# Runki2018/litehandnet

Hardware: AMD Instinct MI355X
Metric: images/sec fwd+bwd @256x256 bs64 litehandnet (higher is better)
Workload: dtype f32; 1 GPU; litehandnet variant B (MSRB hourglass litehourglass.py) C=128, 256x256x3 -> 21x64x64, per-GPU batch 64, train-mode BN, fwd + TopdownHeatmapLoss + bwd + fused Adam; global_batch=64, parallelism=dp1

## Files before the change

### include/lhn.h

```cpp
#ifndef LHN_H
#define LHN_H
#include <stdint.h>
#ifdef __cplusplus
extern "C" {
#endif

#define LHN_VERSION 3
#define LHN_STAT_REPLICAS 32

typedef struct lhn_view {
  float*       data;
  const float* table;
  const float* gate;
  int32_t N, H, W;
  int32_t cstride;
  int32_t coff;
  int32_t C;
  const void* pend;
} lhn_view;

typedef struct lhn_gradview {
  const float* dz;
  const float* dpool;
  const float* coef;
// ... 170 lines not shown
int lhn_shuffle2_fwd(const lhn_view* a, const lhn_view* b, const lhn_view* dst, void* stream);
int lhn_shuffle2_bwd(const lhn_view* a, const lhn_view* b, const lhn_view* dst, const float* ddst, float* da, int acc_a,
                     float* db, int acc_b, void* stream);
int lhn_maxpool2_fwd(const lhn_view* x, const lhn_view* y, void* stream);
int lhn_avgpool_fwd(const lhn_view* x, float* out , int OH, int OW, void* stream);
int lhn_avgpool_fwd2(const lhn_view* x, float* out, int OH, int OW, int out_cstride, int out_coff, void* stream);
int lhn_avgpool_bwd2(const lhn_view* x, const float* dout, int OH, int OW, int out_cstride, int out_coff, float* dx,
                     int dx_accumulate, void* stream);
int lhn_ca_mlp_fwd(const float* pooled , const float* w3 , const float* gamma,
                   const float* beta, float* rmean, float* rvar, int64_t* nbt, const float* w1 ,
                   const float* b1, const float* w2 , const float* b2, const float* dropmask,
                   float* gate, int gate_stride, int gate_coff, float* save , int N, int C,
                   float eps, float momentum, int training, int stage, double* gsum, double count_scale,
                   void* stream);

int lhn_att_mlp_fwd(const float* pooled, const float* gamma, const float* beta, float* rmean, float* rvar,
                    int64_t* nbt, const float* w3 , const float* b3, const float* wl ,
                    const float* bl, const float* dropmask , float* gate, int gate_stride,
                    int gate_coff, float* save, int N, int C, float eps, float momentum, int training, int stage,
                    double* gsum, double count_scale, void* stream);
int lhn_att_mlp_bwd(const float* pooled, const float* gamma, const float* beta, const float* w3, const float* wl,
                    const float* dropmask, float* save, const float* dgate , float* dpool, int cstride,
                    int coff, int H, int W, float* dgamma, float* dbeta, float* dw3, float* db3, float* dwl,
                    float* dbl, int N, int C, int stage, double* gsum, double count_scale, float pgrad_scale,
                    void* stream);

int lhn_se_mlp_fwd(const float* pooled, const float* w1 , const float* b1, const float* w2 ,
                   const float* b2, float* gate, int gate_stride, int gate_coff, float* save, int N, int C, int J,
                   void* stream);
int lhn_se_mlp_fwd2(const float* pooled, const float* w1, const float* b1, const float* w2, const float* b2, float* gate,
                    int gate_stride, int gate_coff, float* save, int N, int C, int J, int mode, void* stream);
int lhn_se_mlp_bwd2(const float* pooled, const float* w1, const float* w2, const float* save, const float* dgate,
                    float* dpool, int cstride, int coff, int H, int W, float* dw1, float* db1, float* dw2, float* db2, int N,
                    int C, int J, int mode, void* stream);
int lhn_se_mlp_bwd(const float* pooled, const float* w1, const float* w2, const float* save, const float* dgate ,
                   float* dpool , int cstride, int coff, int H, int W, float* dw1, float* db1, float* dw2,
                   float* db2, int N, int C, int J, void* stream);

int lhn_bn_bwd_reduce(const lhn_view* y, const lhn_gradview* g, const float* save_mean_invstd,
                      double* sums , const lhn_bnbwdfin* fin , void* stream);
int lhn_bn_bwd_finalize(const double* sums, const float* gamma, const float* save_mean_invstd,
                        float* coef, int cstride, int coff, int C, double count, float* dgamma, float* dbeta,
                        float pgrad_scale , void* stream);
int lhn_bn_bwd_finalize2(const double* sums, const float* gamma, const float* save_mean_invstd, float* coef, int cstride,
                         int coff, int C, int stat_channels, double count, float* dgamma, float* dbeta, float pgrad_scale,
                         void* stream);
int lhn_conv_pw_bwd(const lhn_view* x, const float* w, const lhn_view* y, const lhn_gradview* gy,
                    float* dx , int dx_accumulate, float* dw,
                    float* dbias, int stride, const float* dy_nchw, int nrep, int64_t rep_stride, void* stream);
int lhn_conv_pw_bwd2(const lhn_view* x, const float* w, const lhn_view* y, const lhn_gradview* gy, float* dx,
                     int dx_accumulate, float* dw, float* dbias, int stride, const float* dy_nchw, int nrep, int64_t rep_stride,
                     const lhn_pw_opts* opts, void* stream);
int lhn_conv_dw_bwd(const lhn_view* x, const float* w, const lhn_view* y, const lhn_gradview* gy, float* dx,
                    int dx_accumulate, float* dw, int k, int stride, int pad, int dil, int nrep, int64_t rep_stride,
                    void* stream);
int lhn_conv_dw_bwd2(const lhn_view* x, const float* w, const lhn_view* y, const lhn_gradview* gy, float* dx, int dx_accumulate,
                     float* dw, int k, int stride, int pad, int dil, int nrep, int64_t rep_stride, double* bn_sums,
                     const float* bn_save, int bn_C, int bn_coff, void* stream);
int lhn_conv_dw_bwd3(const lhn_view* x, const float* w, const lhn_view* y, const lhn_gradview* gy, float* dx, int dx_accumulate,
                     float* dw, int k, int stride, int pad, int dil, int nrep, int64_t rep_stride, const float* dx_add0,
                     const float* dx_add1, void* stream);
int lhn_conv_stem_bwd(const float* img, const lhn_view* y, const lhn_gradview* gy, float* dw, int Hi, int Wi,
                      int k, int stride, int pad, int nrep, int64_t rep_stride, void* stream);
int lhn_conv_kxk_bwd(const lhn_view* x, const float* w, const lhn_view* y, const lhn_gradview* gy, float* dx,
                     int dx_accumulate, float* dw, int stride, int nrep, int64_t rep_stride,
                     float* wt_scratch , void* stream);
int lhn_plan_run_range(void* plan, int phase, int64_t step_begin, int64_t step_end, void* workspace,
                       void* const* params, void* const* grads, void* const* io, int training, int grad_replicas,
                       int64_t grad_rep_stride, double count_scale, float pgrad_scale, void* stream);
int lhn_fold_stat_replicas(double* stats, int64_t n, int nrep, void* stream);
int lhn_reduce_replicas(float* out, const float* part, int64_t n, int nrep, int64_t rep_stride, void* stream);
int lhn_ew_bwd(const lhn_view* srcs, int nsrc, const lhn_view* dst, const float* ddst, float out_slope,
               float* const* dsrcs, const int* accumulate, void* stream);
int lhn_ew_bwd2(const lhn_view* src, const lhn_view* dst, const float* ddst, const float* dst_dpool, float out_slope,
                float* dsrc, int accumulate, void* stream);
int lhn_maxpool2_bwd(const lhn_view* x, const lhn_view* y, const float* dy, float* dx, int dx_accumulate,
                     void* stream);
int lhn_maxpool2_bwd2(const lhn_view* x, const lhn_view* y, const float* dy, float* dx, int dx_accumulate, const lhn_bnsum* bns,
                      void* stream);
int lhn_maxpool2_bwd3(const lhn_view* x, const lhn_view* y, const float* dy, float* dx, int dx_accumulate, const lhn_bnsum* bns,
                      const lhn_grad_adds* adds , void* stream);
int lhn_ew_bwd3(const lhn_view* src, const lhn_view* dst, const float* ddst, const float* dst_dpool, float out_slope, float* dsrc,
                int accumulate, const lhn_bnsum* bns, void* stream);
int lhn_ew_bwd_multi(const lhn_view* srcs, int nsrc, const lhn_view* dst, const float* ddst, const float* dst_dpool, float out_slope,
                     float* const* dsrcs, const int* accumulate, const lhn_bnsum* const* bns, void* stream);
int lhn_avgpool_bwd3(const lhn_view* x, const float* dout, int OH, int OW, int out_cstride, int out_coff, float* dx,
                     int dx_accumulate, const lhn_bnsum* bns, void* stream);
int lhn_conv_pw_bwd3(const lhn_view* x, const float* w, const lhn_view* y, const lhn_gradview* gy, float* dx, int dx_accumulate,
                     float* dw, float* dbias, int stride, const float* dy_nchw, int nrep, int64_t rep_stride,
                     const lhn_pw_opts* opts, const lhn_bnsum* bns , void* stream);
int lhn_conv_dw_bwd4(const lhn_view* x, const float* w, const lhn_view* y, const lhn_gradview* gy, float* dx, int dx_accumulate,
                     float* dw, int k, int stride, int pad, int dil, int nrep, int64_t rep_stride, const lhn_bnsum* bns,
                     const float* dx_add0, const float* dx_add1, const lhn_bnbwdsrc* fin, void* stream);
int lhn_conv_pw_bwd4(const lhn_view* x, const float* w, const lhn_view* y, const lhn_gradview* gy, float* dx, int dx_accumulate,
                     float* dw, float* dbias, int stride, const float* dy_nchw, int nrep, int64_t rep_stride,
                     const lhn_pw_opts* opts, const lhn_bnsum* bns, const lhn_bnbwdsrc* fin, void* stream);
int lhn_avgpool_bwd(const lhn_view* x, const float* dout , int OH, int OW, float* dx,
                    int dx_accumulate, void* stream);
int lhn_gate_bwd_reduce(const lhn_view* y, const float* dz, float* dgate , void* stream);
typedef struct lhn_bn_slices {
  const float* save[2];
  double*      sums[2];
  int32_t      lo[2], C[2];
  int32_t      n;
} lhn_bn_slices;
int lhn_gate_bwd_reduce2(const lhn_view* y, const float* dz, float* dgate , float* tsum,
                         const lhn_bn_slices* slices, void* stream);
int lhn_gate_bwd_reduce3(const lhn_view* y, const float* dz, float* dgate, float* tsum, const lhn_bn_slices* slices, int prezeroed,
                         void* stream);
typedef struct lhn_gatesum {
  float*               dgate;
  const lhn_bn_slices* slices;
} lhn_gatesum;
int lhn_conv_pw_bwd5(const lhn_view* x, const float* w, const lhn_view* y, const lhn_gradview* gy, float* dx, int dx_accumulate,
                     float* dw, float* dbias, int stride, const float* dy_nchw, int nrep, int64_t rep_stride,
                     const lhn_pw_opts* opts, const lhn_bnsum* bns, const lhn_bnbwdsrc* fin, const lhn_gatesum* gs, void* stream);
int lhn_avgpool_fwd3(const lhn_view* x, float* out , int OH, int OW, float* pstat ,
                     const lhn_bn_slices* slices, void* stream);
int lhn_ca_mlp_bwd2(const float* pooled, const float* w3, const float* gamma, const float* w1, const float* w2,
                    const float* dropmask, const float* save, const float* dgate, float* dpool, int cstride, int coff, int H,
                    int W, float* dw3, float* dgamma, float* dbeta, float* dw1, float* db1, float* dw2, float* db2, int N, int C,
                    int stage, double* gsum, double count_scale, float pgrad_scale, const float* tsum, const float* pstat,
                    const lhn_bn_slices* slices, void* stream);
int lhn_avgpool_fwd4(const lhn_view* x, float* out, int OH, int OW, float* pstat, const lhn_bn_slices* slices,
                     const lhn_view* copy_src, void* stream);
int lhn_ca_mlp_bwd(const float* pooled, const float* w3, const float* gamma, const float* w1, const float* w2,
                   const float* dropmask, const float* save, const float* dgate, float* dpool ,
                   int cstride, int coff, int H, int W, float* dw3, float* dgamma, float* dbeta, float* dw1,
                   float* db1, float* dw2, float* db2, int N, int C, int stage, double* gsum, double count_scale,
                   float pgrad_scale, void* stream);

int lhn_cbam_layout(int N, int H, int W, int C, int64_t* save_off , int64_t* scratch_off );
int lhn_cbam_fwd(const lhn_view* p, const lhn_view* r, const float* w1, const float* w2, const float* w7, const lhn_view* out,
                 float* save, void* stream);
int lhn_cbam_bwd(const lhn_view* p, const lhn_view* r, const float* w1, const float* w2, const float* w7, const lhn_view* out,
                 const float* dout, float* dp, float* dr, float* dw1, float* dw2, float* dw7, const float* save, float* scratch,
                 void* stream);

int lhn_adam_step(float* param, const float* grad, float* exp_avg, float* exp_avg_sq, int64_t n, double lr, double beta1,
                  double beta2, double eps, double weight_decay, int64_t step, void* stream);

typedef struct lhn_op {
  int32_t kind;
  int32_t in_buf[3], in_coff[3], in_C[3];
  int32_t reserved[6];
  int32_t out_buf, out_coff, out_C;
  int32_t p[12];
  int64_t ws[12];
  int32_t i[8];
  float   f[8];
} lhn_op;

typedef struct lhn_buf {
  int64_t data_off, table_off, gate_off, grad_off, dpool_off, coef_off;
  int32_t N, H, W, C;
} lhn_buf;

void* lhn_plan_create(const lhn_buf* bufs, int nbufs, const lhn_op* fwd, int nfwd, const lhn_op* bwd, int nbwd);
void  lhn_plan_destroy(void* plan);
int   lhn_plan_head_gate_fold(void* plan);
#define LHN_RUN_TABLES_CURRENT 2
#define LHN_RUN_GRAPH 4
int   lhn_plan_run(void* plan, int phase, void* workspace, void* const* params, void* const* grads,
                   void* const* io, int training, int grad_replicas, int64_t grad_rep_stride, void* stream);

#ifdef __cplusplus
}
#endif
#endif
```

### litehandnet_amd/_lib.py

```python
import ctypes as C
import os

import torch

_HERE = os.path.dirname(os.path.abspath(__file__))
LIB_PATH = os.path.join(_HERE, "liblhn.so")
_lib = None


class LhnError(RuntimeError):
    pass


class View(C.Structure):
    _fields_ = [("data", C.c_void_p), ("table", C.c_void_p), ("gate", C.c_void_p),
                ("N", C.c_int32), ("H", C.c_int32), ("W", C.c_int32),
                ("cstride", C.c_int32), ("coff", C.c_int32), ("C", C.c_int32), ("pend", C.c_void_p)]


class GradView(C.Structure):
    _fields_ = [("dz", C.c_void_p), ("dpool", C.c_void_p), ("coef", C.c_void_p)]


class Op(C.Structure):
    _fields_ = [("kind", C.c_int32),
                ("in_buf", C.c_int32 * 3), ("in_coff", C.c_int32 * 3), ("in_C", C.c_int32 * 3), ("reserved", C.c_int32 * 6),
                ("out_buf", C.c_int32), ("out_coff", C.c_int32), ("out_C", C.c_int32),
                ("p", C.c_int32 * 12), ("ws", C.c_int64 * 12), ("i", C.c_int32 * 8), ("f", C.c_float * 8)]


class Buf(C.Structure):
    _fields_ = [("data_off", C.c_int64), ("table_off", C.c_int64), ("gate_off", C.c_int64),
                ("grad_off", C.c_int64), ("dpool_off", C.c_int64), ("coef_off", C.c_int64),
                ("N", C.c_int32), ("H", C.c_int32), ("W", C.c_int32), ("C", C.c_int32)]


SYMBOLS = [
    "lhn_version", "lhn_deterministic", "lhn_last_error", "lhn_device_ok",
    "lhn_heatmap_encode", "lhn_heatmap_argmax", "lhn_heatmap_refine", "lhn_transform_preds",
    "lhn_heatmap_decode", "lhn_heatmap_decode_dark", "lhn_heatmap_decode_dark_udp", "lhn_heatmap_nms", "lhn_heatmap_topk", "lhn_pck_accuracy",
    "lhn_eval_state_bytes", "lhn_eval_accumulate", "lhn_eval_finalize",
    "lhn_loss_balanced_mse_fwd", "lhn_loss_balanced_mse_bwd", "lhn_affine_warp_normalize", "lhn_affine_warp_normalize2", "lhn_random_flip", "lhn_hsv_jitter", "lhn_simdr_encode", "lhn_simdr_loss_fwd", "lhn_simdr_loss_bwd",
    "lhn_conv_pw_fwd", "lhn_conv_pw_fwd2", "lhn_conv_pw_bwd2", "lhn_conv_dw_fwd", "lhn_conv_dw_fwd2", "lhn_conv_dw_fwd3", "lhn_conv_pw_dw3_fwd", "lhn_conv_dw3_pw_fwd", "lhn_msrb_round_scratch_bytes", "lhn_msrb_round_fwd", "lhn_bottleneck_fwd", "lhn_conv_stem_fwd", "lhn_conv_kxk_fwd",
    "lhn_bn_finalize", "lhn_table_fill", "lhn_table_bias", "lhn_fold_bn", "lhn_ew_fwd", "lhn_ew_fwd2", "lhn_ew_fwd3", "lhn_ew_mul_bwd", "lhn_bilinear_bwd", "lhn_shuffle2_fwd", "lhn_shuffle2_bwd", "lhn_bn_finalize2", "lhn_bn_bwd_finalize2", "lhn_maxpool2_fwd", "lhn_avgpool_fwd", "lhn_avgpool_fwd2", "lhn_avgpool_bwd2", "lhn_se_mlp_fwd2", "lhn_se_mlp_bwd2", "lhn_ca_mlp_fwd", "lhn_att_mlp_fwd", "lhn_att_mlp_bwd", "lhn_se_mlp_fwd", "lhn_se_mlp_bwd",
    "lhn_bn_bwd_reduce", "lhn_bn_bwd_finalize", "lhn_conv_pw_bwd", "lhn_conv_dw_bwd", "lhn_conv_dw_bwd2", "lhn_conv_dw_bwd3", "lhn_conv_dw_bwd4", "lhn_conv_pw_bwd4", "lhn_conv_pw_bwd5", "lhn_plan_head_gate_fold", "lhn_conv_stem_bwd",
    "lhn_conv_kxk_bwd", "lhn_ew_bwd", "lhn_ew_bwd2", "lhn_maxpool2_bwd", "lhn_maxpool2_bwd2", "lhn_maxpool2_bwd3", "lhn_ew_bwd3", "lhn_ew_bwd_multi", "lhn_avgpool_bwd3", "lhn_conv_pw_bwd3", "lhn_avgpool_bwd", "lhn_gate_bwd_reduce", "lhn_gate_bwd_reduce2", "lhn_gate_bwd_reduce3", "lhn_adam_step", "lhn_avgpool_fwd3", "lhn_avgpool_fwd4", "lhn_ca_mlp_bwd2",
    "lhn_ca_mlp_bwd", "lhn_reduce_replicas", "lhn_fold_stat_replicas", "lhn_plan_create", "lhn_plan_destroy", "lhn_plan_run", "lhn_plan_run_range",
    "lhn_cbam_layout", "lhn_cbam_fwd", "lhn_cbam_bwd",
]


def lib():
    global _lib
    if _lib is None:
        if not os.path.exists(LIB_PATH):
            raise LhnError(f"{LIB_PATH} is missing: run `python -m litehandnet_amd.build` "
                           "(hipcc --offload-arch=gfx950); there is no CPU fallback")
        _lib = C.CDLL(LIB_PATH)
        _lib.lhn_last_error.restype = C.c_char_p
        _lib.lhn_plan_create.restype = C.c_void_p
        _lib.lhn_plan_destroy.restype = None
        _lib.lhn_eval_state_bytes.restype = C.c_int64
        _lib.lhn_conv_dw3_pw_fwd.argtypes = [C.c_void_p, C.c_void_p, C.c_int, C.c_void_p, C.c_void_p, C.c_void_p, C.c_void_p, C.c_void_p]
        _lib.lhn_conv_dw3_pw_fwd.restype = C.c_int
        _lib.lhn_msrb_round_scratch_bytes.argtypes = [C.c_int, C.c_int, C.c_int, C.c_int]
        _lib.lhn_msrb_round_scratch_bytes.restype = C.c_int64
        _lib.lhn_msrb_round_fwd.argtypes = [C.c_void_p, C.c_void_p, C.c_void_p, C.c_void_p, C.c_void_p, C.c_void_p, C.c_void_p, C.c_int, C.c_int,
                                            C.c_void_p, C.c_void_p]
        _lib.lhn_msrb_round_fwd.restype = C.c_int
        _lib.lhn_bottleneck_fwd.argtypes = [C.c_void_p, C.c_int] + [C.c_void_p] * 8 + [C.c_float, C.c_void_p, C.c_void_p, C.c_void_p]
        _lib.lhn_bottleneck_fwd.restype = C.c_int
        _lib.lhn_cbam_layout.argtypes = [C.c_int, C.c_int, C.c_int, C.c_int, C.c_void_p, C.c_void_p]
        _lib.lhn_cbam_layout.restype = C.c_int
        _lib.lhn_cbam_fwd.argtypes = [C.c_void_p] * 8
        _lib.lhn_cbam_fwd.restype = C.c_int
        _lib.lhn_cbam_bwd.argtypes = [C.c_void_p] * 15
        _lib.lhn_cbam_bwd.restype = C.c_int
    return _lib


def cbam_layout(N, H, W, Cc):
    sv, sc = (C.c_int64 * 10)(), (C.c_int64 * 8)()
    check(lib().lhn_cbam_layout(N, H, W, Cc, sv, sc), "lhn_cbam_layout")
    return list(sv), list(sc)


def check(status, what=""):
    if status != 0:
        raise LhnError(f"{what}: status {status}: {lib().lhn_last_error().decode()}")


def require_device(t=None):
    if not torch.cuda.is_available():
        raise LhnError("no GPU visible: litehandnet_amd has no CPU fallback")
    if t is not None and not t.is_cuda:
        raise LhnError("tensor must live on the GPU (litehandnet_amd has no CPU fallback)")


def ptr(t):
    return C.c_void_p(0) if t is None else C.c_void_p(t.data_ptr())


def stream():
    return C.c_void_p(torch.cuda.current_stream().cuda_stream)


def f32c(t, name="tensor"):
    require_device(t)
    if t.dtype != torch.float32:
        t = t.float()
    return t.contiguous()
```

### litehandnet_amd/csrc/k_conv_head.hip

```cpp
#include <stdlib.h>
#include "lhn_common.h"

bool lhn_head_stream_on() {
  static int v = -1;
  if (v < 0) {
    const char* e = getenv("LHN_HEAD_STREAM");
    v = (e && e[0] == '0') ? 0 : 1;
  }
  return v == 1;
}

constexpr int HCIN = 128, HLDX = HCIN + 4;
constexpr int HLDR = HCIN + 8;

__global__ void __launch_bounds__(256, 2) k_head_fwd(lhn_view x, const float* __restrict__ w, const float* __restrict__ bias,
                                                     float* __restrict__ y_nchw, int cout, int M, int HoWo, int ntiles, int64_t bstride) {
  constexpr int BM = 128, C4 = HCIN / 4, RP = 256 / C4, PF = BM / RP;
  extern __shared__ __attribute__((aligned(16))) float smem[];
  const int tid = threadIdx.x, lane = tid & 63, wave = __builtin_amdgcn_readfirstlane(tid >> 6), l31 = lane & 31, lh = lane >> 5;
  const int co = l31;
  float wreg[HCIN / 2];
#pragma unroll
  for (int kc = 0; kc < HCIN / 8; ++kc) {
    f4 v = (f4){0.f, 0.f, 0.f, 0.f};
    if (co < cout) v = *reinterpret_cast<const f4*>(w + (int64_t)co * HCIN + kc * 8 + 4 * lh);
    wreg[kc * 4 + 0] = v.x; wreg[kc * 4 + 1] = v.y; wreg[kc * 4 + 2] = v.z; wreg[kc * 4 + 3] = v.w;
  }
  const float bv = (bias && co < cout) ? bias[co] : 0.f;
  const int c4 = tid % C4, row0 = tid / C4, cabs = x.coff + 4 * c4;
  const bool uni = HoWo % BM == 0;
  const f4 one4 = (f4){1.f, 1.f, 1.f, 1.f};
  f4 pre[PF], gpre = one4;
  auto issue = [&](int tile) __attribute__((always_inline)) {
#pragma unroll
    for (int p = 0; p < PF; ++p) {
      const int m = min(tile * BM + row0 + p * RP, M - 1);
      pre[p] = *reinterpret_cast<const f4*>(x.data + (int64_t)m * x.cstride + cabs);
    }
    if (uni) gpre = x.gate ? *reinterpret_cast<const f4*>(x.gate + (int64_t)(min(tile * BM, M - 1) / HoWo) * x.cstride + cabs) : one4;
  };
  int tile = blockIdx.x;
  if (tile < ntiles) issue(tile);
  const Xf4 xf = lhn_load_xf(x, cabs);
  for (; tile < ntiles; tile += gridDim.x) {
#pragma unroll
    for (int p = 0; p < PF; ++p) {
      const int row = row0 + p * RP, m = tile * BM + row;
      f4 g = gpre;
      if (!uni) g = x.gate ? *reinterpret_cast<const f4*>(x.gate + (int64_t)(min(m, M - 1) / HoWo) * x.cstride + cabs) : one4;
      const f4 v = lhn_apply_xf(pre[p], xf) * g;
      *reinterpret_cast<f4*>(smem + row * HLDX + 4 * c4) = m < M ? v : (f4){0.f, 0.f, 0.f, 0.f};
    }
    __syncthreads();
    if (tile + (int)gridDim.x < ntiles) issue(tile + gridDim.x);
    f16v acc;
#pragma unroll
    for (int r = 0; r < 16; ++r) acc[r] = 0.f;
    const float* arow = smem + (wave * 32 + l31) * HLDX + 4 * lh;
#pragma unroll
    for (int kc = 0; kc < HCIN / 8; ++kc) {
      const f4 a = *reinterpret_cast<const f4*>(arow + kc * 8);
      acc = __builtin_amdgcn_mfma_f32_32x32x2f32(a.x, wreg[kc * 4 + 0], acc, 0, 0, 0);
      acc = __builtin_amdgcn_mfma_f32_32x32x2f32(a.y, wreg[kc * 4 + 1], acc, 0, 0, 0);
      acc = __builtin_amdgcn_mfma_f32_32x32x2f32(a.z, wreg[kc * 4 + 2], acc, 0, 0, 0);
      acc = __builtin_amdgcn_mfma_f32_32x32x2f32(a.w, wreg[kc * 4 + 3], acc, 0, 0, 0);
    }
    __syncthreads();
    if (co < cout) {
      const int mbase = tile * BM + wave * 32 + 4 * lh;
#pragma unroll
      for (int g = 0; g < 4; ++g) {
        const int m0 = mbase + 8 * g;
        if (m0 < M) {
          const int n = m0 / HoWo, p = m0 - n * HoWo;
          *reinterpret_cast<f4*>(y_nchw + (int64_t)n * bstride + (int64_t)co * HoWo + p) =
              (f4){acc[4 * g] + bv, acc[4 * g + 1] + bv, acc[4 * g + 2] + bv, acc[4 * g + 3] + bv};
        }
      }
    }
  }
}

int lhn_head_fwd(const lhn_view* x, const float* w, const float* bias, float* y_nchw, int cout, int HoWo, int64_t bstride, hipStream_t s) {
  const int M = x->N * HoWo, ntiles = (M + 127) / 128;
  const size_t lds = (size_t)128 * HLDX * sizeof(float);
  static LhnKernelCfg cfg;
  int per_cu = 1;
  if (!lhn_kernel_cfg(cfg, &k_head_fwd, lds, 2, &per_cu)) {
    lhn_set_error("lhn_conv_pw_fwd: cannot reserve %zu B of LDS", lds);
    return 2;
  }
  int grid = lhn_num_cus() * per_cu;
  if (grid > ntiles) grid = ntiles;
  hipLaunchKernelGGL(k_head_fwd, dim3(grid), dim3(256), lds, s, *x, w, bias, y_nchw, cout, M, HoWo, ntiles, bstride);
  return 0;
}

struct HeadGate {
  float* dgate;
  float* tsum;
  const float* save[2];
  int lo[2], C[2], n;
};

template <bool GS>
__global__ void __launch_bounds__(256, 2) k_head_bwd(lhn_view x, const float* __restrict__ w, const float* __restrict__ dy,
                                                     float* __restrict__ dx, int dx_acc, float* __restrict__ dw, float* __restrict__ dbias,
                                                     int cout, int M, int HoWo, int ntiles, int chunk, int64_t bstride, int nrep,
                                                     int64_t rep_stride, HeadGate hg) {
  constexpr int PX = 64, LDY = 36, XC4 = HCIN / 4, XRP = 256 / XC4, XPF = PX / XRP;
  extern __shared__ __attribute__((aligned(16))) float smem[];
  float* dYs = smem;
  float* Xs = dYs + PX * LDY;
  float* Xr = Xs + PX * HLDX;
  const int tid = threadIdx.x, lane = tid & 63, wave = __builtin_amdgcn_readfirstlane(tid >> 6), l31 = lane & 31, lh = lane >> 5;
  const int xc4 = tid % XC4, xr0 = tid / XC4, xabs = x.coff + 4 * xc4;
  const int yr4 = tid & 15, yco = tid >> 4;
  const bool uni = HoWo % PX == 0;
  const f4 one4 = (f4){1.f, 1.f, 1.f, 1.f}, zero4 = (f4){0.f, 0.f, 0.f, 0.f};
  f4 xraw[XPF], yraw[2], gpre = one4;
  auto issue = [&](int tile) __attribute__((always_inline)) {
#pragma unroll
    for (int p = 0; p < XPF; ++p) {
      const int m = min(tile * PX + xr0 + p * XRP, M - 1);
      xraw[p] = *reinterpret_cast<const f4*>(x.data + (int64_t)m * x.cstride + xabs);
    }
    const int m4 = min(tile * PX + 4 * yr4, M - 4);
    const int n = m4 / HoWo, p = m4 - n * HoWo;
#pragma unroll
    for (int k = 0; k < 2; ++k)
      yraw[k] = yco + 16 * k < cout ? *reinterpret_cast<const f4*>(dy + (int64_t)n * bstride + (int64_t)(yco + 16 * k) * HoWo + p) : zero4;
    if (uni) gpre = x.gate ? *reinterpret_cast<const f4*>(x.gate + (int64_t)(min(tile * PX, M - 1) / HoWo) * x.cstride + xabs) : one4;
  };
  const int t0 = blockIdx.x * chunk, t1 = min(ntiles, t0 + chunk);
  if (t0 < t1) issue(t0);
  const Xf4 xf = lhn_load_xf(x, xabs);
  float wreg[16];
#pragma unroll
  for (int k = 0; k < 16; ++k) {
    const int co = (k >> 2) * 8 + 4 * lh + (k & 3);
    wreg[k] = (dx && co < cout) ? w[(int64_t)co * HCIN + 32 * wave + l31] : 0.f;
  }
  f16v accw;
#pragma unroll
  for (int r = 0; r < 16; ++r) accw[r] = 0.f;
  double bsum[2] = {0.0, 0.0};
  const int cg = x.coff + 32 * wave + l31;
  float g_sc = 1.f, g_sh = 0.f, g_sl = 1.f, g_mean = 0.f, g_inv = 1.f, g_d = 0.f, g_0 = 0.f, g_1 = 0.f;
  int n_cur = -1;
  if (GS) {
    if (x.table) {
      g_sc = x.table[cg];
      g_sh = x.table[x.cstride + cg];
      g_sl = x.table[2 * x.cstride + cg];
    }
#pragma unroll
    for (int k = 0; k < 2; ++k)
      if (k < hg.n && cg >= hg.lo[k] && cg < hg.lo[k] + hg.C[k]) {
        g_mean = hg.save[k][cg - hg.lo[k]];
        g_inv = hg.save[k][hg.C[k] + cg - hg.lo[k]];
      }
  }
  auto gflush = [&]() __attribute__((always_inline)) {
    const float sd = g_d + __shfl_xor(g_d, 32, 64), s0 = g_0 + __shfl_xor(g_0, 32, 64), s1 = g_1 + __shfl_xor(g_1, 32, 64);
    if (lh == 0 && n_cur >= 0) {
      atomicAdd(hg.dgate + (int64_t)n_cur * x.cstride + cg, sd);
      atomicAdd(hg.tsum + ((int64_t)n_cur * 2 + 0) * x.cstride + cg, s0);
      atomicAdd(hg.tsum + ((int64_t)n_cur * 2 + 1) * x.cstride + cg, s1);
    }
    g_d = g_0 = g_1 = 0.f;
  };

  for (int tile = t0; tile < t1; ++tile) {
#pragma unroll
    for (int p = 0; p < XPF; ++p) {
      const int row = xr0 + p * XRP, m = tile * PX + row;
      f4 g = gpre;
      if (!uni) g = x.gate ? *reinterpret_cast<const f4*>(x.gate + (int64_t)(min(m, M - 1) / HoWo) * x.cstride + xabs) : one4;
      const f4 v = lhn_apply_xf(xraw[p], xf) * g;
      *reinterpret_cast<f4*>(Xs + row * HLDX + 4 * xc4) = m < M ? v : zero4;
      if (GS) *reinterpret_cast<f4*>(Xr + row * HLDR + 4 * xc4) = m < M ? xraw[p] : zero4;
    }
    const bool yin = tile * PX + 4 * yr4 < M;
#pragma unroll
    for (int k = 0; k < 2; ++k) {
      const f4 v = yin ? yraw[k] : zero4;
// ... 30 lines not shown
          accx = __builtin_amdgcn_mfma_f32_32x32x2f32(a.y, wreg[kc * 4 + 1], accx, 0, 0, 0);
          accx = __builtin_amdgcn_mfma_f32_32x32x2f32(a.z, wreg[kc * 4 + 2], accx, 0, 0, 0);
          accx = __builtin_amdgcn_mfma_f32_32x32x2f32(a.w, wreg[kc * 4 + 3], accx, 0, 0, 0);
        }
        if (GS) {
          const float* xr = Xr + (hh * 32 + 4 * lh) * HLDR + 32 * wave + l31;
#pragma unroll
          for (int r = 0; r < 16; ++r) {
            const float raw = xr[((r & 3) + 8 * (r >> 2)) * HLDR];
            const float u = raw * g_sc + g_sh;
            const float da = accx[r] * (u > 0.f ? 1.f : g_sl);
            g_d += accx[r] * lhn_lrelu(u, g_sl);
            g_0 += da;
            g_1 += da * ((raw - g_mean) * g_inv);
          }
        }
        const int cs = x.cstride, mbase = tile * PX + hh * 32 + 4 * lh;
        float* o = dx + (int64_t)mbase * cs + cg;
        if (tile * PX + PX <= M) {
          if (dx_acc) {
#pragma unroll
            for (int r = 0; r < 16; ++r) o[((r & 3) + 8 * (r >> 2)) * cs] += accx[r];
          } else {
#pragma unroll
            for (int r = 0; r < 16; ++r) o[((r & 3) + 8 * (r >> 2)) * cs] = accx[r];
          }
        } else {
#pragma unroll
          for (int r = 0; r < 16; ++r) {
            const int ro = (r & 3) + 8 * (r >> 2);
            if (mbase + ro < M) o[(int64_t)ro * cs] = dx_acc ? o[(int64_t)ro * cs] + accx[r] : accx[r];
          }
        }
      }
    }
    __syncthreads();
  }
  if (GS) gflush();
  if (t0 >= t1) return;
  float* rep = dw + (size_t)(blockIdx.x % nrep) * rep_stride;
#pragma unroll
  for (int r = 0; r < 16; ++r) {
    const int co = (r & 3) + 8 * (r >> 2) + 4 * lh;
    if (co < cout) atomicAdd(rep + (int64_t)co * HCIN + 32 * wave + l31, accw[r]);
  }
  if (dbias) {
#pragma unroll
    for (int k = 0; k < 2; ++k) {
      double v = bsum[k];
      v += __shfl_xor(v, 1, 64);
      v += __shfl_xor(v, 2, 64);
      v += __shfl_xor(v, 4, 64);
      v += __shfl_xor(v, 8, 64);
      if (yr4 == 0 && yco + 16 * k < cout) atomicAdd(dbias + (size_t)(blockIdx.x % nrep) * rep_stride + yco + 16 * k, (float)v);
    }
  }
}

template <bool GS>
static int launch_head_bwd(const lhn_view* x, const float* w, const float* dy, float* dx, int dx_acc, float* dw, float* dbias, int cout,
                           int HoWo, int64_t bstride, int nrep, int64_t rep_stride, const HeadGate& hg, hipStream_t s) {
  const int M = x->N * HoWo, ntiles = (M + 63) / 64;
  const size_t lds = (size_t)(64 * 36 + 64 * HLDX + (GS ? 64 * HLDR : 0)) * sizeof(float);
  static LhnKernelCfg cfg;
  int per_cu = 1;
  if (!lhn_kernel_cfg(cfg, &k_head_bwd<GS>, lds, 2, &per_cu)) {
    lhn_set_error("lhn_conv_pw_bwd: cannot reserve %zu B of LDS", lds);
    return 2;
  }
  int grid = lhn_num_cus() * per_cu;
  if (grid > ntiles) grid = ntiles;
  const int chunk = (ntiles + grid - 1) / grid;
  grid = (ntiles + chunk - 1) / chunk;
  hipLaunchKernelGGL(k_head_bwd<GS>, dim3(grid), dim3(256), lds, s, *x, w, dy, dx, dx_acc, dw, dbias, cout, M, HoWo, ntiles, chunk, bstride,
                     nrep, rep_stride, hg);
  return 0;
}

int lhn_head_bwd(const lhn_view* x, const float* w, const float* dy, float* dx, int dx_acc, float* dw, float* dbias, int cout, int HoWo,
                 int64_t bstride, int nrep, int64_t rep_stride, const lhn_gatesum* gs, hipStream_t s) {
  HeadGate hg;
  memset(&hg, 0, sizeof(hg));
  if (!gs) return launch_head_bwd<false>(x, w, dy, dx, dx_acc, dw, dbias, cout, HoWo, bstride, nrep, rep_stride, hg, s);
  hg.dgate = gs->dgate;
  hg.tsum = gs->dgate + (size_t)x->N * x->cstride;
  if (gs->slices)
    for (int k = 0; k < gs->slices->n; ++k) {
      hg.save[hg.n] = gs->slices->save[k];
      hg.lo[hg.n] = gs->slices->lo[k];
      hg.C[hg.n] = gs->slices->C[k];
      ++hg.n;
    }
  return launch_head_bwd<true>(x, w, dy, dx, dx_acc, dw, dbias, cout, HoWo, bstride, nrep, rep_stride, hg, s);
}
```

### litehandnet_amd/csrc/k_conv_pw.hip

```cpp
#include <stdlib.h>
#include "lhn_common.h"

struct PwGeom {
  int wstride, kvalid, wrows, yacc, statC;
  int64_t nchw_bstride;
};

template <int CIN>
__device__ __forceinline__ void pw_stage_w(float* Ws, int LDA, const float* __restrict__ w, int rows_pad, const PwGeom& g) {
  constexpr int C4 = CIN / 4;
  const bool vec = (g.wstride % 4 == 0) && (g.kvalid % 4 == 0) && ((reinterpret_cast<uintptr_t>(w) & 15) == 0);
  for (int i = threadIdx.x; i < rows_pad * C4; i += 256) {
    const int co = i / C4, k4 = i % C4;
    f4 v = (f4){0.f, 0.f, 0.f, 0.f};
    if (co < g.wrows) {
      const float* r = w + (int64_t)co * g.wstride + k4 * 4;
      if (vec) {
        if (4 * k4 < g.kvalid) v = *reinterpret_cast<const f4*>(r);
      } else {
        if (4 * k4 + 0 < g.kvalid) v.x = r[0];
        if (4 * k4 + 1 < g.kvalid) v.y = r[1];
        if (4 * k4 + 2 < g.kvalid) v.z = r[2];
        if (4 * k4 + 3 < g.kvalid) v.w = r[3];
      }
// ... 827 lines not shown
    if (tl < T) {
      const int it = tl / NTI, jt = tl % NTI;
#pragma unroll
      for (int r = 0; r < 16; ++r) {
        const int co = 32 * it + (r & 3) + 8 * (r >> 2) + 4 * lh;
        if (co < geo.wrows && 32 * jt + l31 < geo.kvalid) atomicAdd(dw + (int64_t)co * geo.wstride + 32 * jt + l31, accw[t][r]);
      }
    }
  }
  if (dbias) {
    if (NCHW) {
    } else {
      f4* bred = reinterpret_cast<f4*>(dYs);
      bred[yr0 * YC4 + yc4] = ych_ok ? bsum : (f4){0.f, 0.f, 0.f, 0.f};
      __syncthreads();
      if (tid < YC4 && 4 * tid < cout) {
        f4 t = (f4){0.f, 0.f, 0.f, 0.f};
        for (int j = 0; j < YRP; ++j) t += bred[j * YC4 + tid];
        float* db = dbias + (size_t)(blockIdx.x % nrep) * rep_stride + 4 * tid;
        if (4 * tid + 0 < geo.wrows) atomicAdd(db + 0, t.x);
        if (4 * tid + 1 < geo.wrows) atomicAdd(db + 1, t.y);
        if (4 * tid + 2 < geo.wrows) atomicAdd(db + 2, t.z);
        if (4 * tid + 3 < geo.wrows) atomicAdd(db + 3, t.w);
      }
    }
  }
}

__global__ void __launch_bounds__(256) k_bias_grad_nchw(const float* __restrict__ dy, float* __restrict__ db, int N, int C,
                                                        int HW, int64_t bstride) {
  const int co = blockIdx.x;
  double s = 0;
  for (int n = blockIdx.y; n < N; n += gridDim.y) {
    const float* p = dy + (int64_t)n * bstride + (int64_t)co * HW;
    float a = 0.f;
    for (int i = threadIdx.x; i < HW; i += blockDim.x) a += p[i];
    s += a;
  }
  s = lhn_wave_sum_d(s);
  __shared__ double red[4];
  if ((threadIdx.x & 63) == 0) red[threadIdx.x >> 6] = s;
  __syncthreads();
  if (threadIdx.x == 0) atomicAdd(db + co, (float)(red[0] + red[1] + red[2] + red[3]));
}

template <int CIN, int NTO, bool NCHW, bool BNS = false>
static int launch_pw_bwd_t(const lhn_view* x, const float* w, const lhn_view* y, const lhn_gradview* gy, float* dx, int dx_acc,
                         float* dw, float* dbias, int stride, const float* dy_nchw, int cout, int nrep, int64_t rep_stride,
                         const PwGeom& geo, hipStream_t s, const lhn_bnsum& bs) {
  const int M = y->N * y->H * y->W;
  const int ntiles = (M + 63) / 64;
  constexpr int COP = 32 * NTO;
  const size_t lds = (size_t)(COP * (CIN + 4) + 64 * (COP + 4) + 64 * (CIN + 4)) * sizeof(float);
  static LhnKernelCfg cfg;
  int per_cu = 1;
  if (!lhn_kernel_cfg(cfg, &k_pw_bwd<CIN, NTO, NCHW, BNS>, lds, 4, &per_cu)) {
    lhn_set_error("lhn_conv_pw_bwd: cannot reserve %zu B of LDS", lds);
    return 2;
  }
  int grid = lhn_num_cus() * per_cu;
  if (grid > ntiles) grid = ntiles;
  lhn_gradview g = *gy;
  hipLaunchKernelGGL((k_pw_bwd<CIN, NTO, NCHW, BNS>), dim3(grid), dim3(256), lds, s, *x, w, *y, g, dx, dx_acc, dw, dbias, stride, dy_nchw,
                     cout, M, ntiles, nrep, rep_stride, geo, bs);
  if (dbias && dy_nchw)
    hipLaunchKernelGGL(k_bias_grad_nchw, dim3(geo.wrows, lhn_deterministic_mode() ? 1 : (y->N < 16 ? y->N : 16)), dim3(256), 0, s, dy_nchw, dbias, y->N, cout,
                       y->H * y->W, geo.nchw_bstride);
  return 0;
}

template <int CIN, int NTO>
static int launch_pw_bwd(const lhn_view* x, const float* w, const lhn_view* y, const lhn_gradview* gy, float* dx, int dx_acc,
                         float* dw, float* dbias, int stride, const float* dy_nchw, int cout, int nrep, int64_t rep_stride,
                         const PwGeom& geo, hipStream_t s, const lhn_bnsum& bs) {
  if (dy_nchw) return launch_pw_bwd_t<CIN, NTO, true>(x, w, y, gy, dx, dx_acc, dw, dbias, stride, dy_nchw, cout, nrep, rep_stride, geo, s, bs);
  if constexpr (CIN * NTO * 32 < 64 * 128) {
    if (bs.sums && dx && stride == 1)
      return launch_pw_bwd_t<CIN, NTO, false, true>(x, w, y, gy, dx, dx_acc, dw, dbias, stride, dy_nchw, cout, nrep, rep_stride, geo, s, bs);
  }
  if (bs.sums) return -1;
  return launch_pw_bwd_t<CIN, NTO, false>(x, w, y, gy, dx, dx_acc, dw, dbias, stride, dy_nchw, cout, nrep, rep_stride, geo, s, bs);
}

template <int CIN, int COUT, int PX, int PF, bool DYST, bool BNS, int OCC>
__global__ void __launch_bounds__(256, OCC) k_pw_bwd_wr(lhn_view x, const float* __restrict__ w, lhn_view y, lhn_gradview gy,
                                                        float* __restrict__ dx, int dx_acc, float* __restrict__ dw, float* __restrict__ dbias,
                                                        int M, int ntiles, int nrep, int64_t rep_stride, lhn_bnsum bs, lhn_bnbwdsrc fs) {
  constexpr int NTI = CIN / 32, NTO = COUT / 32, LDY = COUT + 4, LDX = CIN + 4;
  constexpr bool ONE = NTI == 1;
  constexpr int NDW = ONE ? 1 : NTO * NTI / 4;
  constexpr int KW = ONE ? 32 : PX;
  constexpr int NDX = (NTI == 4 && PX == 64) ? 2 : 1;
  constexpr int NWC = 4 / NTI;
  static_assert(ONE ? (NTO == 1 && PX == 128) : ((NTI == 2 || NTI == 4) && (NTO == 2 || NTO == 4) && (PX == 64 || (PX == 32 && NTI == 4))),
                "32 -> 32 at 128 pixels; 64 / 128 channels on either side at 64 (or 32) pixels");
  static_assert(!BNS || NDX == 1, "reader-side sums: one dX sub-tile per wave");
  extern __shared__ __attribute__((aligned(16))) float smem[];
  float* dYs = smem;
  float* Xs = dYs + PX * LDY;
  float* xt = Xs + PX * LDX;
  float* yt = xt + 3 * CIN;
  float* cf = yt + 3 * COUT;
  float* Xr = cf + 3 * COUT;
  const int tid = threadIdx.x, lane = tid & 63, wave = __builtin_amdgcn_readfirstlane(tid >> 6), l31 = lane & 31, lh = lane >> 5;
  const int HoWo = y.H * y.W;
  float* dzw = const_cast<float*>(gy.dz);

  constexpr int XC4 = CIN / 4, XRP = 256 / XC4, XPF = PX / XRP;
  constexpr int YC4 = COUT / 4, YRP = 256 / YC4, YPF = PX / YRP;
  constexpr int ZCH = YPF < 4 ? YPF : 4;
  const int xc4 = tid % XC4, xr0 = tid / XC4, xabs = x.coff + 4 * xc4;
  const int yc4 = tid % YC4, yr0 = tid / YC4, yabs = y.coff + 4 * yc4;

  f4 xraw[XPF], yraw[YPF], ydz[YPF];
  auto issue = [&](int tile) __attribute__((always_inline)) {
#pragma unroll
    for (int p = 0; p < XPF; ++p) {
      const int m = min(tile * PX + xr0 + p * XRP, M - 1);
      xraw[p] = *reinterpret_cast<const f4*>(x.data + (int64_t)m * x.cstride + xabs);
    }
#pragma unroll
    for (int p = 0; p < YPF; ++p) {
      const int m = min(tile * PX + yr0 + p * YRP, M - 1);
      if (PF >= 1) yraw[p] = *reinterpret_cast<const f4*>(y.data + (int64_t)m * y.cstride + yabs);
      if (PF >= 2) ydz[p] = *reinterpret_cast<const f4*>(gy.dz + (int64_t)m * y.cstride + yabs);
    }
  };
  f4 bsum = (f4){0.f, 0.f, 0.f, 0.f};
  auto commit = [&](int tile) __attribute__((always_inline)) {
    Xf4 xxf;
    xxf.sc = *reinterpret_cast<const f4*>(xt + 4 * xc4);
    xxf.sh = *reinterpret_cast<const f4*>(xt + CIN + 4 * xc4);
    xxf.sl = *reinterpret_cast<const f4*>(xt + 2 * CIN + 4 * xc4);
#pragma unroll
    for (int p = 0; p < XPF; ++p) {
      const int row = xr0 + p * XRP, m = tile * PX + row;
      f4 v = (f4){0.f, 0.f, 0.f, 0.f};
      if (m < M) {
        v = lhn_apply_xf(xraw[p], xxf);
        if (!BNS && x.gate) v *= *reinterpret_cast<const f4*>(x.gate + (int64_t)(m / HoWo) * x.cstride + xabs);
      }
      *reinterpret_cast<f4*>(Xs + row * LDX + 4 * xc4) = v;
      if (BNS) *reinterpret_cast<f4*>(Xr + row * CIN + 4 * xc4) = m < M ? xraw[p] : (f4){0.f, 0.f, 0.f, 0.f};
    }
    Xf4 yxf;
    Gr4 ygr;
    yxf.sc = *reinterpret_cast<const f4*>(yt + 4 * yc4);
    yxf.sh = *reinterpret_cast<const f4*>(yt + COUT + 4 * yc4);
    yxf.sl = *reinterpret_cast<const f4*>(yt + 2 * COUT + 4 * yc4);
    ygr.A = *reinterpret_cast<const f4*>(cf + 4 * yc4);
    ygr.B = *reinterpret_cast<const f4*>(cf + COUT + 4 * yc4);
    ygr.Cc = *reinterpret_cast<const f4*>(cf + 2 * COUT + 4 * yc4);
#pragma unroll
    for (int p = 0; p < YPF; ++p) {
      if (PF < 2 && p % ZCH == 0) {
#pragma unroll
        for (int q = p; q < p + ZCH; ++q) {
          const int mq = min(tile * PX + yr0 + q * YRP, M - 1);
          if (PF < 1) yraw[q] = *reinterpret_cast<const f4*>(y.data + (int64_t)mq * y.cstride + yabs);
          ydz[q] = *reinterpret_cast<const f4*>(gy.dz + (int64_t)mq * y.cstride + yabs);
        }
      }
      const int row = yr0 + p * YRP, m = tile * PX + row;
      f4 v = (f4){0.f, 0.f, 0.f, 0.f};
      if (m < M) {
        int n = 0, h = 0, ww = 0;
        if (y.gate || gy.dpool) {
          n = m / HoWo;
          const int r = m - n * HoWo;
          h = r / y.W;
          ww = r - h * y.W;
        }
        const f4 du = lhn_grad_du(y, gy, yxf, yraw[p], ydz[p], n, h, ww, yabs);
        v = ygr.A * du + ygr.B * yraw[p] + ygr.Cc;
        bsum += v;
        if (DYST) *reinterpret_cast<f4*>(dzw + (int64_t)m * y.cstride + yabs) = v;
      }
      *reinterpret_cast<f4*>(dYs + row * LDY + 4 * yc4) = v;
    }
  };

  int tile = blockIdx.x;
  if (tile < ntiles) issue(tile);
  static_assert(PX * LDY * sizeof(float) >= 2 * LHN_FIN_THREADS * sizeof(double), "dYs holds the replica fold's partials");
  LhnBwdPre fpre;
  if (fs.sums) {
    fpre = lhn_bn_bwd_pre(fs, 0, COUT);
    lhn_bn_bwd_fold_part_ct<COUT>(fs.sums, fs.stat_channels, reinterpret_cast<double*>(dYs));
  }
  for (int i = tid; i < CIN; i += 256) {
    xt[i] = x.table ? x.table[x.coff + i] : 1.f;
    xt[CIN + i] = x.table ? x.table[x.cstride + x.coff + i] : 0.f;
    xt[2 * CIN + i] = x.table ? x.table[2 * x.cstride + x.coff + i] : 1.f;
  }
  for (int i = tid; i < COUT; i += 256) {
    yt[i] = y.table ? y.table[y.coff + i] : 1.f;
    yt[COUT + i] = y.table ? y.table[y.cstride + y.coff + i] : 0.f;
    yt[2 * COUT + i] = y.table ? y.table[2 * y.cstride + y.coff + i] : 1.f;
    if (fs.sums) continue;
    cf[i] = gy.coef ? gy.coef[y.coff + i] : 1.f;
    cf[COUT + i] = gy.coef ? gy.coef[y.cstride + y.coff + i] : 0.f;
    cf[2 * COUT + i] = gy.coef ? gy.coef[2 * y.cstride + y.coff + i] : 0.f;
  }
  const int jt = NTI == 4 ? wave : NTI == 2 ? wave >> 1 : 0;
  const int mt0 = NTI == 4 ? 0 : NTI == 2 ? (wave & 1) : wave;
  float wreg[COUT / 2];
#pragma unroll
  for (int k = 0; k < COUT / 2; ++k) wreg[k] = dx ? w[(int64_t)((k >> 2) * 8 + 4 * lh + (k & 3)) * CIN + 32 * jt + l31] : 0.f;
  f16v accw[NDW];
#pragma unroll
  for (int t = 0; t < NDW; ++t)
#pragma unroll
    for (int r = 0; r < 16; ++r) accw[t][r] = 0.f;
  float b_sc = 1.f, b_sh = 0.f, b_sl = 1.f, b_mean = 0.f, b_inv = 0.f, b_s = 0.f, b_q = 0.f;
  if (BNS) {
    const int ci = 32 * jt + l31;
    if (x.table) {
      b_sc = x.table[x.coff + ci];
      b_sh = x.table[x.cstride + x.coff + ci];
      b_sl = x.table[2 * x.cstride + x.coff + ci];
    }
    b_mean = bs.save[bs.coff + ci];
    b_inv = bs.save[bs.C + bs.coff + ci];
  }
  double* const bst = BNS ? bs.sums + (size_t)(blockIdx.x % LHN_STAT_REPLICAS) * 2 * bs.C + bs.coff + (tid & (CIN - 1)) : nullptr;
  const int bsC = BNS ? bs.C : 0;
  if (fs.sums) {
    __syncthreads();
    if (tid < COUT)
      lhn_bn_bwd_coef_put(lhn_bn_bwd_coef(reinterpret_cast<const double*>(dYs), COUT, LHN_FIN_THREADS / COUT, tid, fpre.gamma, fpre.mean,
                                          fpre.inv, fs.count),
                          fs, const_cast<float*>(gy.coef), y.cstride, y.coff, tid, cf, COUT, tid, blockIdx.x == 0);
  }
  __syncthreads();

  for (; tile < ntiles; tile += gridDim.x) {
    commit(tile);
    __syncthreads();
    if (tile + (int)gridDim.x < ntiles) issue(tile + gridDim.x);
    {
      const float* ap = dYs + ((ONE ? 32 * wave : 0) + lh) * LDY + l31 + (ONE ? 0 : 32 * (wave / NTI));
      const float* bp = Xs + ((ONE ? 32 * wave : 0) + lh) * LDX + l31 + (ONE ? 0 : 32 * (wave % NTI));
#pragma unroll 4
      for (int ks = 0; ks < KW / 2; ++ks) {
        const float b = bp[(2 * ks) * LDX];
        float a[NDW];
#pragma unroll
        for (int t = 0; t < NDW; ++t) a[t] = ap[(2 * ks) * LDY + 32 * (4 / NTI) * t];
#pragma unroll
        for (int t = 0; t < NDW; ++t) accw[t] = __builtin_amdgcn_mfma_f32_32x32x2f32(a[t], b, accw[t], 0, 0, 0);
      }
    }
    if (dx) {
      f16v accx[NDX];
#pragma unroll
      for (int hh = 0; hh < NDX; ++hh)
#pragma unroll
        for (int r = 0; r < 16; ++r) accx[hh][r] = 0.f;
      const float* arow = dYs + (mt0 * 32 + l31) * LDY + 4 * lh;
#pragma unroll
      for (int kc = 0; kc < COUT / 8; ++kc) {
#pragma unroll
        for (int hh = 0; hh < NDX; ++hh) {
          const f4 a = *reinterpret_cast<const f4*>(arow + hh * 32 * LDY + kc * 8);
          accx[hh] = __builtin_amdgcn_mfma_f32_32x32x2f32(a.x, wreg[kc * 4 + 0], accx[hh], 0, 0, 0);
          accx[hh] = __builtin_amdgcn_mfma_f32_32x32x2f32(a.y, wreg[kc * 4 + 1], accx[hh], 0, 0, 0);
          accx[hh] = __builtin_amdgcn_mfma_f32_32x32x2f32(a.z, wreg[kc * 4 + 2], accx[hh], 0, 0, 0);
          accx[hh] = __builtin_amdgcn_mfma_f32_32x32x2f32(a.w, wreg[kc * 4 + 3], accx[hh], 0, 0, 0);
        }
      }
      const int cs = x.cstride;
#pragma unroll
      for (int hh = 0; hh < NDX; ++hh) {
        const int mbase = tile * PX + (mt0 + hh) * 32 + 4 * lh;
        float* o = dx + (int64_t)mbase * cs + x.coff + 32 * jt + l31;
        if (BNS) {
          const float* xr = Xr + ((mt0 + hh) * 32 + 4 * lh) * CIN + 32 * jt + l31;
#pragma unroll
          for (int r = 0; r < 16; ++r) {
            const float raw = xr[((r & 3) + 8 * (r >> 2)) * CIN];
            const float du = accx[hh][r] * (raw * b_sc + b_sh > 0.f ? 1.f : b_sl);
            b_s += du;
            b_q += du * ((raw - b_mean) * b_inv);
          }
        }
        if (tile * PX + PX <= M) {
          if (dx_acc) {
#pragma unroll
            for (int r = 0; r < 16; ++r) o[((r & 3) + 8 * (r >> 2)) * cs] += accx[hh][r];
          } else {
#pragma unroll
            for (int r = 0; r < 16; ++r) o[((r & 3) + 8 * (r >> 2)) * cs] = accx[hh][r];
          }
        } else if constexpr (BNS) {
          float* ot = dx + (int64_t)(tile * PX + (mt0 + hh) * 32) * cs + x.coff + 32 * jt + l31;
#pragma unroll
          for (int r = 0; r < 16; ++r) {
            const int ro = (r & 3) + 8 * (r >> 2) + 4 * lh;
            if (tile * PX + (mt0 + hh) * 32 + ro < M) ot[(int64_t)ro * cs] = dx_acc ? ot[(int64_t)ro * cs] + accx[hh][r] : accx[hh][r];
          }
        } else {
#pragma unroll
          for (int r = 0; r < 16; ++r) {
            const int ro = (r & 3) + 8 * (r >> 2);
            if (mbase + ro < M) o[ro * cs] = dx_acc ? o[ro * cs] + accx[hh][r] : accx[hh][r];
          }
        }
      }
    }
    __syncthreads();
  }

  if (BNS) {
    float* bred = Xs;
    const float ss = b_s + __shfl_xor(b_s, 32, 64), qq = b_q + __shfl_xor(b_q, 32, 64);
    if (lh == 0) {
      bred[((jt * NWC + mt0) * 2 + 0) * 32 + l31] = ss;
      bred[((jt * NWC + mt0) * 2 + 1) * 32 + l31] = qq;
    }
    __syncthreads();
    if (tid < CIN) {
      const int jc = tid >> 5, c = tid & 31;
      double ds = 0.0, dq = 0.0;
#pragma unroll
      for (int v = 0; v < NWC; ++v) {
        ds += (double)bred[((jc * NWC + v) * 2 + 0) * 32 + c];
        dq += (double)bred[((jc * NWC + v) * 2 + 1) * 32 + c];
      }
      atomicAdd(bst, ds);
      atomicAdd(bst + bsC, dq);
    }
  }
  dw += (size_t)(blockIdx.x % nrep) * rep_stride;
  if constexpr (ONE) {
    float* wred = dYs;
#pragma unroll
    for (int r = 0; r < 16; ++r) wred[(wave * 16 + r) * 64 + lane] = accw[0][r];
    __syncthreads();
#pragma unroll
    for (int q = 0; q < 4; ++q) {
      const int r = 4 * q + wave, co = (r & 3) + 8 * (r >> 2) + 4 * lh;
      const float v = ((wred[r * 64 + lane] + wred[(16 + r) * 64 + lane]) + wred[(32 + r) * 64 + lane]) + wred[(48 + r) * 64 + lane];
      atomicAdd(dw + (int64_t)co * CIN + l31, v);
    }
    if (dbias) __syncthreads();
  } else {
#pragma unroll
    for (int t = 0; t < NDW; ++t) {
      const int it = wave / NTI + (4 / NTI) * t, jw = wave % NTI;
#pragma unroll
      for (int r = 0; r < 16; ++r) {
        const int co = 32 * it + (r & 3) + 8 * (r >> 2) + 4 * lh;
        atomicAdd(dw + (int64_t)co * CIN + 32 * jw + l31, accw[t][r]);
      }
    }
  }
  if (dbias) {
    f4* bred = reinterpret_cast<f4*>(dYs);
    bred[yr0 * YC4 + yc4] = bsum;
    __syncthreads();
    if (tid < YC4) {
      f4 t = (f4){0.f, 0.f, 0.f, 0.f};
      for (int j = 0; j < YRP; ++j) t += bred[j * YC4 + tid];
      float* db = dbias + (size_t)(blockIdx.x % nrep) * rep_stride + 4 * tid;
      atomicAdd(db + 0, t.x);
      atomicAdd(db + 1, t.y);
      atomicAdd(db + 2, t.z);
      atomicAdd(db + 3, t.w);
    }
  }
}

template <int CIN, int COUT, int PX, int PF, bool DYST = true, bool BNS = false, int OCC = 2>
static int launch_pw_bwd_wr(const lhn_view* x, const float* w, const lhn_view* y, const lhn_gradview* gy, float* dx, int dx_acc, float* dw,
                            float* dbias, int nrep, int64_t rep_stride, hipStream_t s, const lhn_bnsum& bs, const lhn_bnbwdsrc* fsp = nullptr) {
  const int M = y->N * y->H * y->W, ntiles = (M + PX - 1) / PX;
  lhn_bnbwdsrc fs;
  if (fsp) fs = *fsp; else memset(&fs, 0, sizeof(fs));
  const size_t lds = (size_t)(PX * (COUT + 4) + PX * (CIN + 4) + 3 * CIN + 6 * COUT + (BNS ? PX * CIN : 0)) * sizeof(float);
  static LhnKernelCfg cfg;
  int per_cu = 1;
  if (!lhn_kernel_cfg(cfg, &k_pw_bwd_wr<CIN, COUT, PX, PF, DYST, BNS, OCC>, lds, OCC, &per_cu)) {
    lhn_set_error("lhn_conv_pw_bwd: cannot reserve %zu B of LDS", lds);
    return 2;
  }
  int grid = lhn_num_cus() * per_cu;
  if (grid > ntiles) grid = ntiles;
  hipLaunchKernelGGL((k_pw_bwd_wr<CIN, COUT, PX, PF, DYST, BNS, OCC>), dim3(grid), dim3(256), lds, s, *x, w, *y, *gy, dx, dx_acc, dw, dbias,
                     M, ntiles, nrep, rep_stride, bs, fs);
  return 0;
}

static bool pw_bwd_narrow_off() {
  static int off = -1;
  if (off < 0) {
    const char* e = getenv("LHN_PW_BWD_NARROW");
    off = (e && e[0] == '0') ? 1 : 0;
  }
  return off == 1;
}

static bool pw_bwd_split_forced() {
  static int on = -1;
  if (on < 0) {
    const char* e = getenv("LHN_PW_BWD_SPLIT");
    on = (e && e[0] == '1') ? 1 : 0;
  }
  return on == 1;
}

int lhn_pw_bwd_split(const lhn_view* x, const float* w, const lhn_view* y, const lhn_gradview* gy, float* dx, int dx_accumulate,
                     float* dw, float* dbias, int nrep, int64_t rep_stride, hipStream_t s);

extern "C" int lhn_conv_pw_bwd2(const lhn_view* x, const float* w, const lhn_view* y, const lhn_gradview* gy, float* dx,
                                int dx_accumulate, float* dw, float* dbias, int stride, const float* dy_nchw, int nrep,
                                int64_t rep_stride, const lhn_pw_opts* opts, void* stream) {
  return lhn_conv_pw_bwd3(x, w, y, gy, dx, dx_accumulate, dw, dbias, stride, dy_nchw, nrep, rep_stride, opts, nullptr, stream);
}
extern "C" int lhn_conv_pw_bwd3(const lhn_view* x, const float* w, const lhn_view* y, const lhn_gradview* gy, float* dx,
                                int dx_accumulate, float* dw, float* dbias, int stride, const float* dy_nchw, int nrep,
                                int64_t rep_stride, const lhn_pw_opts* opts, const lhn_bnsum* bns, void* stream) {
  return lhn_conv_pw_bwd4(x, w, y, gy, dx, dx_accumulate, dw, dbias, stride, dy_nchw, nrep, rep_stride, opts, bns, nullptr, stream);
}
extern "C" int lhn_conv_pw_bwd4(const lhn_view* x, const float* w, const lhn_view* y, const lhn_gradview* gy, float* dx,
                                int dx_accumulate, float* dw, float* dbias, int stride, const float* dy_nchw, int nrep,
                                int64_t rep_stride, const lhn_pw_opts* opts, const lhn_bnsum* bns, const lhn_bnbwdsrc* fin, void* stream) {
  return lhn_conv_pw_bwd5(x, w, y, gy, dx, dx_accumulate, dw, dbias, stride, dy_nchw, nrep, rep_stride, opts, bns, fin, nullptr, stream);
}
static int pw_bwd_run(const lhn_view* x, const float* w, const lhn_view* y, const lhn_gradview* gy, float* dx, int dx_accumulate, float* dw,
                      float* dbias, int stride, const float* dy_nchw, int nrep, int64_t rep_stride, const lhn_pw_opts* opts,
                      const lhn_bnsum* bns, const lhn_bnbwdsrc* fin, const lhn_gatesum* gs, bool* gs_done, void* stream);
extern "C" int lhn_conv_pw_bwd5(const lhn_view* x, const float* w, const lhn_view* y, const lhn_gradview* gy, float* dx,
                                int dx_accumulate, float* dw, float* dbias, int stride, const float* dy_nchw, int nrep,
                                int64_t rep_stride, const lhn_pw_opts* opts, const lhn_bnsum* bns, const lhn_bnbwdsrc* fin,
                                const lhn_gatesum* gs, void* stream) {
  if (gs && !gs->dgate) gs = nullptr;
  if (gs) LHN_CHECK_ARG(lhn_view_ok(x) && dx && !dx_accumulate && stride == 1 && (!gs->slices || (gs->slices->n >= 0 && gs->slices->n <= 2)),
                        "lhn_conv_pw_bwd5: gate sums need a stored dx (no accumulate), stride 1 and 0..2 BatchNorm slices");
  bool gs_done = false;
  const int rc = pw_bwd_run(x, w, y, gy, dx, dx_accumulate, dw, dbias, stride, dy_nchw, nrep, rep_stride, opts, bns, fin, gs, &gs_done, stream);
  if (rc || !gs || gs_done) return rc;
  lhn_view xv = *x;
  xv.gate = nullptr;
  return lhn_gate_bwd_reduce3(&xv, dx, gs->dgate, gs->dgate + (size_t)x->N * x->cstride, gs->slices, 1, stream);
}
static int pw_bwd_run(const lhn_view* x, const float* w, const lhn_view* y, const lhn_gradview* gy, float* dx, int dx_accumulate, float* dw,
                      float* dbias, int stride, const float* dy_nchw, int nrep, int64_t rep_stride, const lhn_pw_opts* opts,
                      const lhn_bnsum* bns, const lhn_bnbwdsrc* fin, const lhn_gatesum* gs, bool* gs_done, void* stream) {
  if (nrep < 1) nrep = 1;
  if (fin && !fin->sums) fin = nullptr;
  lhn_bnsum bs;
  memset(&bs, 0, sizeof(bs));
  if (bns && bns->sums) {
    LHN_CHECK_ARG(x && y && bns->save && dx && stride == 1 && x->C <= 128 && y->C <= 128 && x->C * y->C < 64 * 128 && !x->gate && x->table &&
                      bns->coff >= 0 && bns->coff + x->C <= bns->C,
                  "lhn_conv_pw_bwd3: BatchNorm sums ride in the fused kernel only (stride 1, Cin * Cout < 8192, ungated input inside the producer's channels)");
    bs = *bns;
  }
  LHN_CHECK_ARG(lhn_view_ok(x) && w && y && gy && dw && lhn_no_pend(x) && lhn_no_pend(y), "lhn_conv_pw_bwd: bad view / null pointer");
  LHN_CHECK_ARG(stride == 1 || stride == 2, "lhn_conv_pw_bwd: stride %d", stride);
  LHN_CHECK_ARG(stride == 1 || !dx || dx_accumulate, "lhn_conv_pw_bwd: stride-2 dgrad only accumulates into a zeroed gradient");
  if (!dy_nchw) LHN_CHECK_ARG(lhn_view_ok(y) && gy->dz, "lhn_conv_pw_bwd: bad output view / missing dz");
  const int Cout = y->C, Cin = x->C, HoWo = y->H * y->W;
  const int wcols = (opts && opts->w_cols > 0) ? opts->w_cols : Cin, wrows = (opts && opts->w_rows > 0) ? opts->w_rows : Cout;
  LHN_CHECK_ARG(wcols <= Cin && wcols > Cin - 4 && wrows <= Cout, "lhn_conv_pw_bwd: weight [%d][%d] does not fit views %d -> %d",
                wrows, wcols, Cin, Cout);
  const int64_t bstride = (opts && opts->nchw_batch_stride > 0) ? opts->nchw_batch_stride : (int64_t)Cout * HoWo;
  hipStream_t s = (hipStream_t)stream;
  const bool wr_wide = !bs.sums && stride == 1 && !dy_nchw && wcols == Cin && wrows == Cout && !pw_bwd_split_forced() && !pw_wr_off() &&
                       ((Cin == 128 && Cout == 128) || (Cin == 64 && Cout == 128) || (Cin == 128 && Cout == 64));
  const bool wr_narrow = stride == 1 && !dy_nchw && wcols == Cin && wrows == Cout && Cin == Cout && (Cin == 64 || Cin == 32) &&
                         !pw_bwd_narrow_off() && !pw_wr_off();
  if (dy_nchw && lhn_head_stream_on() && !pw_wr_off() && stride == 1 && !bs.sums && !fin && Cin == HEAD_CIN && wcols == Cin && Cout <= 32 && wrows == Cout &&
      HoWo % 4 == 0 && bstride % 4 == 0 && (!gs || (HoWo % 64 == 0 && !lhn_deterministic_mode())) &&
      ((reinterpret_cast<uintptr_t>(dy_nchw) | reinterpret_cast<uintptr_t>(x->data)) & 15) == 0) {
    const int rc = lhn_head_bwd(x, w, dy_nchw, dx, dx_accumulate, dw, dbias, Cout, HoWo, bstride, nrep, rep_stride, gs, s);
    if (rc) return rc;
    LHN_CHECK_LAUNCH("lhn_conv_pw_bwd");
    *gs_done = gs != nullptr;
    return 0;
  }
  if (fin) {
    LHN_CHECK_ARG(!dy_nchw && gy->coef && fin->save_mean_invstd && fin->count > 0 && fin->stat_channels >= Cout,
                  "lhn_conv_pw_bwd4: finalize source needs gy->coef, saved statistics and stat_channels >= Cout");
    if (!wr_wide && !wr_narrow) {
      const int rc = lhn_bn_bwd_finalize2(fin->sums, fin->gamma, fin->save_mean_invstd, const_cast<float*>(gy->coef), y->cstride, y->coff,
                                          Cout, fin->stat_channels, fin->count, fin->dgamma, fin->dbeta, fin->pgrad_scale, stream);
      if (rc) return rc;
      fin = nullptr;
    }
  }
  if (wr_wide) {
    int rc = -1;
    if (Cin == 128 && Cout == 128) rc = launch_pw_bwd_wr<128, 128, 32, 1>(x, w, y, gy, dx, dx_accumulate, dw, dbias, nrep, rep_stride, s, bs, fin);
    else if (Cin == 64 && Cout == 128) rc = launch_pw_bwd_wr<64, 128, 64, 1>(x, w, y, gy, dx, dx_accumulate, dw, dbias, nrep, rep_stride, s, bs, fin);
    else if (Cin == 128 && Cout == 64) rc = launch_pw_bwd_wr<128, 64, 64, 2>(x, w, y, gy, dx, dx_accumulate, dw, dbias, nrep, rep_stride, s, bs, fin);
    if (rc == 0) {
      LHN_CHECK_LAUNCH("lhn_conv_pw_bwd");
      return 0;
    }
    if (rc > 0) return rc;
  }
  if (wr_narrow) {
    int rc;
    if (Cin == 64) rc = bs.sums ? launch_pw_bwd_wr<64, 64, 64, 2, false, true>(x, w, y, gy, dx, dx_accumulate, dw, dbias, nrep, rep_stride, s, bs, fin)
                                : launch_pw_bwd_wr<64, 64, 64, 2, false, false>(x, w, y, gy, dx, dx_accumulate, dw, dbias, nrep, rep_stride, s, bs, fin);
    else rc = bs.sums ? launch_pw_bwd_wr<32, 32, 128, 2, false, true>(x, w, y, gy, dx, dx_accumulate, dw, dbias, nrep, rep_stride, s, bs, fin)
                      : launch_pw_bwd_wr<32, 32, 128, 2, false, false, 3>(x, w, y, gy, dx, dx_accumulate, dw, dbias, nrep, rep_stride, s, bs, fin);
    if (rc) return rc;
    LHN_CHECK_LAUNCH("lhn_conv_pw_bwd");
    return 0;
  }
  if (!bs.sums && stride == 1 && !dy_nchw && Cin * Cout >= 64 * 128 && Cout % 32 == 0 && Cin % 32 == 0 && Cout <= 256 && wcols == Cin && wrows == Cout) {
    const int rc = lhn_pw_bwd_split(x, w, y, gy, dx, dx_accumulate, dw, dbias, nrep, rep_stride, s);
    if (rc == 0) {
      LHN_CHECK_LAUNCH("lhn_conv_pw_bwd");
      return 0;
    }
    if (rc > 0) return rc;
  }
  for (int co0 = 0; co0 < Cout; co0 += 128) {
    const int cc = Cout - co0 < 128 ? Cout - co0 : 128, nto = (cc + 31) / 32 == 3 ? 4 : (cc + 31) / 32;
    for (int k0 = 0; k0 < Cin; k0 += 128) {
      const int kc = Cin - k0 < 128 ? Cin - k0 : 128, ci = kc <= 32 ? 32 : pw_cin_tile(kc);
      lhn_view xv = *x, yv = *y;
      xv.coff += k0;
      xv.C = kc;
      if (!dy_nchw) {
        yv.coff += co0;
        yv.C = cc;
      }
      PwGeom g;
      g.wstride = wcols;
      g.kvalid = wcols - k0 < kc ? wcols - k0 : kc;
      g.wrows = wrows - co0 < cc ? (wrows - co0 < 0 ? 0 : wrows - co0) : cc;
      g.yacc = 0;
      g.statC = Cout;
      g.nchw_bstride = bstride;
      const float* wv = w + (int64_t)co0 * wcols + k0;
      float* dwv = dw + (int64_t)co0 * wcols + k0;
      float* dbv = (dbias && k0 == 0) ? dbias + co0 : nullptr;
      const float* dyv = dy_nchw ? dy_nchw + (int64_t)co0 * HoWo : nullptr;
      const int acc = dx_accumulate || co0 > 0;
      int rc = -1;
#define PWB_CASE(CI, NTV) \
  if (ci == CI && nto == NTV) rc = launch_pw_bwd<CI, NTV>(&xv, wv, &yv, gy, dx, acc, dwv, dbv, stride, dyv, cc, nrep, rep_stride, g, s, bs);
      PWB_CASE(32, 1) PWB_CASE(32, 2) PWB_CASE(32, 4) PWB_CASE(64, 1) PWB_CASE(64, 2) PWB_CASE(64, 4) PWB_CASE(128, 1)
      PWB_CASE(128, 2) PWB_CASE(128, 4)
#undef PWB_CASE
      LHN_CHECK_ARG(rc != -1, "lhn_conv_pw_bwd: unsupported channels Cin=%d Cout=%d", Cin, Cout);
      if (rc) return rc;
    }
  }
  LHN_CHECK_LAUNCH("lhn_conv_pw_bwd");
  return 0;
}

extern "C" int lhn_conv_pw_bwd(const lhn_view* x, const float* w, const lhn_view* y, const lhn_gradview* gy, float* dx,
                               int dx_accumulate, float* dw, float* dbias, int stride, const float* dy_nchw, int nrep,
                               int64_t rep_stride, void* stream) {
  return lhn_conv_pw_bwd2(x, w, y, gy, dx, dx_accumulate, dw, dbias, stride, dy_nchw, nrep, rep_stride, nullptr, stream);
}
```

### litehandnet_amd/csrc/k_misc.hip

```cpp
#include "lhn_common.h"

static inline int grid_cap(int64_t blocks, int cap_per_cu) {
  const int64_t cap = (int64_t)lhn_num_cus() * cap_per_cu;
  if (blocks > cap) blocks = cap;
  if (blocks < 1) blocks = 1;
  return (int)blocks;
}
static inline bool pow2i(int v) { return v > 0 && (v & (v - 1)) == 0; }

__global__ void __launch_bounds__(LHN_FIN_THREADS) k_bn_finalize(const double* __restrict__ stats, const float* __restrict__ gamma,
                              const float* __restrict__ beta, float* __restrict__ rmean, float* __restrict__ rvar,
                              int64_t* __restrict__ nbt, float* __restrict__ table, int cs, int coff, int C,
                              float* __restrict__ save, double count, float eps, float momentum, float slope, int training,
                              const float* __restrict__ cbias, int SC) {
  __shared__ double part[2 * LHN_FIN_THREADS];
  const int nt = blockDim.x;
  int G = nt / C;
  G = G < 1 ? 1 : (G > LHN_STAT_REPLICAS ? LHN_STAT_REPLICAS : G);
  for (int c0 = 0; c0 < C; c0 += nt) {
    const int g = threadIdx.x / C, c = c0 + (G > 1 ? threadIdx.x - g * C : threadIdx.x);
    if (c0) __syncthreads();
    if (training && g < G && c < C) {
      double s1 = 0, s2 = 0;
#pragma unroll 4
// ... 116 lines not shown
      for (int w0 = LHN_LANE0(pl, PL); w0 < dst.W; w0 += 4 * PL) {
        f4 raw[3][4];
#pragma unroll
        for (int k = 0; k < 3; ++k)
          if (k < nsrc) {
            const lhn_view& v = S.v[k];
#pragma unroll
            for (int j = 0; j < 4; ++j) {
              const int w = min(w0 + j * PL, dst.W - 1);
              const int ws = (v.W == dst.W) ? w : nearest_src(w, v.W, dst.W);
              raw[k][j] = *reinterpret_cast<const f4*>(base[k] + (size_t)ws * v.cstride);
            }
          }
#pragma unroll
        for (int j = 0; j < 4; ++j) {
          const int w = w0 + j * PL;
          if (w < dst.W) {
            f4 acc = mul ? (f4){1.f, 1.f, 1.f, 1.f} : (f4){0.f, 0.f, 0.f, 0.f};
#pragma unroll
            for (int k = 0; k < 3; ++k)
              if (k < nsrc) {
                const f4 val = lhn_apply_xf(raw[k][j], xf[k]) * (gate[k] * S.coef[k]);
                if (mul) acc *= val; else acc += val;
              }
            if (out_slope == LHN_SLOPE_RELU_SIGMOID) {
              acc.x = lhn_relu_sigmoid(acc.x); acc.y = lhn_relu_sigmoid(acc.y); acc.z = lhn_relu_sigmoid(acc.z); acc.w = lhn_relu_sigmoid(acc.w);
            } else if (out_slope == LHN_SLOPE_SILU) {
              acc.x = lhn_silu(acc.x); acc.y = lhn_silu(acc.y); acc.z = lhn_silu(acc.z); acc.w = lhn_silu(acc.w);
            } else {
              acc.x = lhn_lrelu(acc.x, out_slope); acc.y = lhn_lrelu(acc.y, out_slope); acc.z = lhn_lrelu(acc.z, out_slope); acc.w = lhn_lrelu(acc.w, out_slope);
            }
            *reinterpret_cast<f4*>(out + (size_t)w * dst.cstride) = acc;
          }
        }
      }
      continue;
    }
    for (int w = LHN_LANE0(pl, PL); w < dst.W; w += PL) {
      f4 acc = mul ? (f4){1.f, 1.f, 1.f, 1.f} : (f4){0.f, 0.f, 0.f, 0.f};
#pragma unroll
      for (int k = 0; k < 3; ++k)
        if (k < nsrc) {
          const lhn_view& v = S.v[k];
          f4 val;
          if (bil && (v.H != dst.H || v.W != dst.W)) {
            int h0, h1, w0, w1;
            float ah, aw;
            bil_taps(h, v.H, dst.H, h0, h1, ah);
            bil_taps(w, v.W, dst.W, w0, w1, aw);
            const float* b0 = v.data + ((size_t)(n * v.H + h0) * v.W) * v.cstride + ca[k];
            const float* b1 = v.data + ((size_t)(n * v.H + h1) * v.W) * v.cstride + ca[k];
            const f4 v00 = lhn_apply_xf(*reinterpret_cast<const f4*>(b0 + (size_t)w0 * v.cstride), xf[k]);
            const f4 v01 = lhn_apply_xf(*reinterpret_cast<const f4*>(b0 + (size_t)w1 * v.cstride), xf[k]);
            const f4 v10 = lhn_apply_xf(*reinterpret_cast<const f4*>(b1 + (size_t)w0 * v.cstride), xf[k]);
            const f4 v11 = lhn_apply_xf(*reinterpret_cast<const f4*>(b1 + (size_t)w1 * v.cstride), xf[k]);
            val = ((v00 * (1.f - aw) + v01 * aw) * (1.f - ah) + (v10 * (1.f - aw) + v11 * aw) * ah) * (gate[k] * S.coef[k]);
          } else {
            const int ws = nearest_src(w, v.W, dst.W);
            val = lhn_apply_xf(*reinterpret_cast<const f4*>(base[k] + (size_t)ws * v.cstride), xf[k]) * (gate[k] * S.coef[k]);
          }
          if (mul) acc *= val; else acc += val;
        }
      if (out_slope == LHN_SLOPE_RELU_SIGMOID) {
        acc.x = lhn_relu_sigmoid(acc.x);
        acc.y = lhn_relu_sigmoid(acc.y);
        acc.z = lhn_relu_sigmoid(acc.z);
        acc.w = lhn_relu_sigmoid(acc.w);
      } else if (out_slope == LHN_SLOPE_SILU) {
        acc.x = lhn_silu(acc.x);
        acc.y = lhn_silu(acc.y);
        acc.z = lhn_silu(acc.z);
        acc.w = lhn_silu(acc.w);
      } else {
        acc.x = lhn_lrelu(acc.x, out_slope);
        acc.y = lhn_lrelu(acc.y, out_slope);
        acc.z = lhn_lrelu(acc.z, out_slope);
        acc.w = lhn_lrelu(acc.w, out_slope);
      }
      *reinterpret_cast<f4*>(out + (size_t)w * dst.cstride) = acc;
    }
  }
}

__global__ void __launch_bounds__(256) k_ew_bwd_src(lhn_view src, lhn_view dst, const float* __restrict__ ddst,
                                                    const float* __restrict__ dst_dpool, float out_slope,
                                                    float* __restrict__ dsrc, int accumulate, lhn_bnsum bs) {
  __shared__ f4 bred[512];
  const int C4 = src.C >> 2, c4 = threadIdx.x % C4, pl = threadIdx.x / C4, PL = 256 / C4;
  f4 bsum = (f4){0.f, 0.f, 0.f, 0.f}, bsq = bsum, bmean = bsum, binv = bsum;
  Xf4 bxf;
  if (bs.sums) {
    bxf = lhn_load_xf(src, src.coff + 4 * c4);
    bmean = *reinterpret_cast<const f4*>(bs.save + bs.coff + 4 * c4);
    binv = *reinterpret_cast<const f4*>(bs.save + bs.C + bs.coff + 4 * c4);
  }
  const int fh = dst.H / src.H, fw = dst.W / src.W;
  const int cd = dst.coff + 4 * c4;
  const int rows = src.N * src.H;
  for (int row = blockIdx.x; row < rows; row += gridDim.x) {
    const int n = row / src.H, h = row - n * src.H;
    const f4 gate = dst.gate ? *reinterpret_cast<const f4*>(dst.gate + (size_t)n * dst.cstride + cd) : (f4){1.f, 1.f, 1.f, 1.f};
    for (int w = LHN_LANE0(pl, PL); w < src.W; w += PL) {
      f4 g = (f4){0.f, 0.f, 0.f, 0.f};
      for (int a = 0; a < fh; ++a)
        for (int b = 0; b < fw; ++b) {
          const int hd = h * fh + a, wd = w * fw + b;
          const size_t pd = ((size_t)(n * dst.H + hd) * dst.W + wd) * dst.cstride + cd;
          f4 e = *reinterpret_cast<const f4*>(ddst + pd) * gate;
          if (dst_dpool) {
            lhn_gradview gv{nullptr, dst_dpool, nullptr};
            e += lhn_dpool_sum(gv, dst, n, hd, wd, cd);
          }
          if (out_slope == LHN_SLOPE_SILU || out_slope == LHN_SLOPE_RELU_SIGMOID) {
            const Xf4 sxf = lhn_load_xf(src, src.coff + 4 * c4);
            const f4 v = lhn_load_val(src, sxf, (int64_t)(n * src.H + h) * src.W + w, n, src.coff + 4 * c4);
            if (out_slope == LHN_SLOPE_SILU) {
              e.x *= lhn_silu_grad(v.x);
              e.y *= lhn_silu_grad(v.y);
              e.z *= lhn_silu_grad(v.z);
              e.w *= lhn_silu_grad(v.w);
            } else {
              e.x *= lhn_relu_sigmoid_grad(v.x);
              e.y *= lhn_relu_sigmoid_grad(v.y);
              e.z *= lhn_relu_sigmoid_grad(v.z);
              e.w *= lhn_relu_sigmoid_grad(v.w);
            }
          } else if (out_slope != 1.f) {
            const f4 o = *reinterpret_cast<const f4*>(dst.data + pd);
            e.x *= o.x > 0.f ? 1.f : out_slope;
            e.y *= o.y > 0.f ? 1.f : out_slope;
            e.z *= o.z > 0.f ? 1.f : out_slope;
            e.w *= o.w > 0.f ? 1.f : out_slope;
          }
          g += e;
        }
      float* o = dsrc + ((size_t)row * src.W + w) * src.cstride + src.coff + 4 * c4;
      if (bs.sums) {
        const f4 raw = *reinterpret_cast<const f4*>(src.data + ((size_t)row * src.W + w) * src.cstride + src.coff + 4 * c4);
        const f4 du = g * lhn_dact_xf(raw, bxf);
        bsum += du;
        bsq += du * ((raw - bmean) * binv);
      }
      if (accumulate) g += *reinterpret_cast<const f4*>(o);
      *reinterpret_cast<f4*>(o) = g;
    }
  }
  if (bs.sums) lhn_bns_flush(bs, bsum, bsq, C4, bred);
}

struct EwBwdMulti {
  int n;
  lhn_view src[3];
  float* dsrc[3];
  int acc[3];
  lhn_bnsum bs[3];
};
__global__ void __launch_bounds__(256) k_ew_bwd_multi(EwBwdMulti m, lhn_view dst, const float* __restrict__ ddst,
                                                      const float* __restrict__ dst_dpool, float out_slope) {
  __shared__ f4 bred[512];
  const int C4 = dst.C >> 2, c4 = threadIdx.x % C4, pl = threadIdx.x / C4, PL = 256 / C4;
  f4 bsum[3], bsq[3], bmean[3], binv[3];
  Xf4 bxf[3];
#pragma unroll
  for (int k = 0; k < 3; ++k) {
    bsum[k] = bsq[k] = bmean[k] = binv[k] = (f4){0.f, 0.f, 0.f, 0.f};
    if (k < m.n && m.bs[k].sums) {
      bxf[k] = lhn_load_xf(m.src[k], m.src[k].coff + 4 * c4);
      bmean[k] = *reinterpret_cast<const f4*>(m.bs[k].save + m.bs[k].coff + 4 * c4);
      binv[k] = *reinterpret_cast<const f4*>(m.bs[k].save + m.bs[k].C + m.bs[k].coff + 4 * c4);
    }
  }
  const int cd = dst.coff + 4 * c4;
  const int rows = dst.N * dst.H;
  for (int row = blockIdx.x; row < rows; row += gridDim.x) {
    const int n = row / dst.H, h = row - n * dst.H;
    const f4 gate = dst.gate ? *reinterpret_cast<const f4*>(dst.gate + (size_t)n * dst.cstride + cd) : (f4){1.f, 1.f, 1.f, 1.f};
    for (int w = LHN_LANE0(pl, PL); w < dst.W; w += PL) {
      const size_t pix = (size_t)row * dst.W + w, pd = pix * dst.cstride + cd;
      f4 e = *reinterpret_cast<const f4*>(ddst + pd) * gate;
      if (dst_dpool) {
        lhn_gradview gv{nullptr, dst_dpool, nullptr};
        e += lhn_dpool_sum(gv, dst, n, h, w, cd);
      }
      if (out_slope != 1.f) {
        const f4 o = *reinterpret_cast<const f4*>(dst.data + pd);
        e.x *= o.x > 0.f ? 1.f : out_slope;
        e.y *= o.y > 0.f ? 1.f : out_slope;
        e.z *= o.z > 0.f ? 1.f : out_slope;
        e.w *= o.w > 0.f ? 1.f : out_slope;
      }
#pragma unroll
      for (int k = 0; k < 3; ++k) {
        if (k < m.n) {
          const size_t ps = pix * m.src[k].cstride + m.src[k].coff + 4 * c4;
          f4 g = e;
          if (m.bs[k].sums) {
            const f4 raw = *reinterpret_cast<const f4*>(m.src[k].data + ps);
            const f4 du = g * lhn_dact_xf(raw, bxf[k]);
            bsum[k] += du;
            bsq[k] += du * ((raw - bmean[k]) * binv[k]);
          }
          float* o = m.dsrc[k] + ps;
          if (m.acc[k]) g += *reinterpret_cast<const f4*>(o);
          *reinterpret_cast<f4*>(o) = g;
        }
      }
    }
  }
#pragma unroll
  for (int k = 0; k < 3; ++k)
    if (k < m.n && m.bs[k].sums) {
      lhn_bns_flush(m.bs[k], bsum[k], bsq[k], C4, bred);
      __syncthreads();
    }
}

__global__ void __launch_bounds__(256) k_maxpool2_fwd(lhn_view x, lhn_view y) {
  const int C4 = y.C >> 2, c4 = threadIdx.x % C4, pl = threadIdx.x / C4, PL = 256 / C4;
  const int ca = x.coff + 4 * c4;
  const Xf4 xf = lhn_load_xf(x, ca);
  const int rows = y.N * y.H;
  for (int row = blockIdx.x; row < rows; row += gridDim.x) {
    const int n = row / y.H, ho = row - n * y.H;
    const f4 gate = x.gate ? *reinterpret_cast<const f4*>(x.gate + (size_t)n * x.cstride + ca) : (f4){1.f, 1.f, 1.f, 1.f};
    for (int wo = LHN_LANE0(pl, PL); wo < y.W; wo += PL) {
      f4 m = (f4){-INFINITY, -INFINITY, -INFINITY, -INFINITY};
#pragma unroll
      for (int o = 0; o < 4; ++o) {
        const int ih = 2 * ho + (o >> 1), iw = 2 * wo + (o & 1);
        if (ih < x.H && iw < x.W) {
// ... 727 lines not shown
  hipLaunchKernelGGL(k_reduce_replicas, dim3(grid_cap((n / 4 + 255) / 256, 8)), dim3(256), 0, (hipStream_t)stream, out, part, n / 4, nrep, rep_stride);
  LHN_CHECK_LAUNCH("lhn_reduce_replicas");
  return 0;
}

int lhn_bn_finalize(const double* stats, const float* gamma, const float* beta, float* running_mean, float* running_var,
                    int64_t* nbt, float* table, int cstride, int coff, int C, float* save, double count, float eps,
                    float momentum, float slope, int training, const float* conv_bias, void* stream) {
  return lhn_bn_finalize2(stats, gamma, beta, running_mean, running_var, nbt, table, cstride, coff, C, C, save, count, eps, momentum,
                          slope, training, conv_bias, stream);
}
int lhn_bn_finalize2(const double* stats, const float* gamma, const float* beta, float* running_mean, float* running_var,
                     int64_t* nbt, float* table, int cstride, int coff, int C, int stat_channels, float* save, double count,
                     float eps, float momentum, float slope, int training, const float* conv_bias, void* stream) {
  LHN_CHECK_ARG(table && C > 0 && coff >= 0 && coff + C <= cstride && stat_channels >= C, "lhn_bn_finalize: bad table slice");
  LHN_CHECK_ARG(training ? (stats != nullptr) : (running_mean && running_var), "lhn_bn_finalize: missing statistics");
  LHN_CHECK_ARG(!training || count >= 1, "lhn_bn_finalize: count");
  int nt = training ? (C >= LHN_FIN_THREADS ? LHN_FIN_THREADS : (LHN_FIN_THREADS / C > LHN_STAT_REPLICAS ? LHN_STAT_REPLICAS : LHN_FIN_THREADS / C) * C)
                    : (C <= 64 ? 64 : (C <= 128 ? 128 : 256));
  nt = (nt + 63) / 64 * 64;
  hipLaunchKernelGGL(k_bn_finalize, dim3(1), dim3(nt), 0, (hipStream_t)stream, stats,
                     gamma, beta, running_mean, running_var, nbt, table, cstride, coff, C, save, count, eps, momentum,
                     slope, training, conv_bias, stat_channels);
  LHN_CHECK_LAUNCH("lhn_bn_finalize");
  return 0;
}

int lhn_table_fill(float* table, int cstride, int coff, int C, float scale, float shift, float slope, void* stream) {
  LHN_CHECK_ARG(table && C > 0 && coff >= 0 && coff + C <= cstride, "lhn_table_fill: bad table slice");
  hipLaunchKernelGGL(k_table_fill, dim3(1), dim3(128), 0, (hipStream_t)stream, table, cstride, coff, C, scale, shift, slope);
  LHN_CHECK_LAUNCH("lhn_table_fill");
  return 0;
}

int lhn_table_bias(float* table, int cstride, int coff, int C, const float* bias, float slope, void* stream) {
  LHN_CHECK_ARG(table && C > 0 && coff >= 0 && coff + C <= cstride, "lhn_table_bias: bad slice");
  hipLaunchKernelGGL(k_table_bias, dim3(1), dim3(128), 0, (hipStream_t)stream, table, cstride, coff, C, bias, slope);
  LHN_CHECK_LAUNCH("lhn_table_bias");
  return 0;
}

int lhn_ew_fwd(const lhn_view* srcs, int nsrc, const lhn_view* dst, float out_slope, void* stream) {
  return lhn_ew_fwd2(srcs, nsrc, nullptr, dst, out_slope, stream);
}
int lhn_ew_fwd2(const lhn_view* srcs, int nsrc, const float* coef, const lhn_view* dst, float out_slope, void* stream) {
  return lhn_ew_fwd3(srcs, nsrc, coef, dst, out_slope, 0, stream);
}
int lhn_ew_fwd3(const lhn_view* srcs, int nsrc, const float* coef, const lhn_view* dst, float out_slope, int mode, void* stream) {
  LHN_CHECK_ARG(srcs && nsrc >= 1 && nsrc <= 3 && lhn_view_ok(dst) && mode >= 0 && mode <= 3, "lhn_ew_fwd: 1..3 sources, valid dst");
  EwSrcs S;
  memset(&S, 0, sizeof(S));
  S.mode = mode;
  for (int i = 0; i < nsrc; ++i) {
    LHN_CHECK_ARG(lhn_view_ok(&srcs[i]) && srcs[i].C == dst->C && srcs[i].N == dst->N && lhn_no_pend(&srcs[i]), "lhn_ew_fwd: source %d mismatch", i);
    S.v[i] = srcs[i];
    S.coef[i] = coef ? coef[i] : 1.f;
  }
  LHN_CHECK_ARG(dst->C % 4 == 0 && dst->C <= 1024, "lhn_ew_fwd: C=%d", dst->C);
  if (S.mode & 2)
    hipLaunchKernelGGL(k_ew_fwd<true>, dim3(grid_cap((int64_t)dst->N * dst->H, 8)), dim3(256), 0, (hipStream_t)stream, S, nsrc, *dst, out_slope);
  else
    hipLaunchKernelGGL(k_ew_fwd<false>, dim3(grid_cap((int64_t)dst->N * dst->H, 8)), dim3(256), 0, (hipStream_t)stream, S, nsrc, *dst, out_slope);
  LHN_CHECK_LAUNCH("lhn_ew_fwd");
  return 0;
}

int lhn_ew_bwd(const lhn_view* srcs, int nsrc, const lhn_view* dst, const float* ddst, float out_slope,
               float* const* dsrcs, const int* accumulate, void* stream) {
  LHN_CHECK_ARG(srcs && nsrc >= 1 && nsrc <= 3 && lhn_view_ok(dst) && ddst && dsrcs && accumulate, "lhn_ew_bwd: bad args");
  for (int i = 0; i < nsrc; ++i) {
    if (!dsrcs[i]) continue;
    const lhn_view* s = &srcs[i];
    LHN_CHECK_ARG(lhn_view_ok(s) && s->C == dst->C, "lhn_ew_bwd: source %d mismatch", i);
    LHN_CHECK_ARG(dst->H % s->H == 0 && dst->W % s->W == 0, "lhn_ew_bwd: non-integer upsample %dx%d -> %dx%d", s->H, s->W, dst->H, dst->W);
    LHN_CHECK_ARG(s->C % 4 == 0 && s->C <= 1024, "lhn_ew_bwd: C=%d", s->C);
    LHN_CHECK_ARG((out_slope != LHN_SLOPE_SILU && out_slope != LHN_SLOPE_RELU_SIGMOID) || (dst->H == s->H && dst->W == s->W),
                  "lhn_ew_bwd: SiLU / ReLU-sigmoid need a single same-size source (source %d)", i);
  }
  for (int i = 0; i < nsrc; ++i) {
    if (!dsrcs[i]) continue;
    const lhn_view* s = &srcs[i];
    lhn_bnsum nob;
    memset(&nob, 0, sizeof(nob));
    hipLaunchKernelGGL(k_ew_bwd_src, dim3(grid_cap((int64_t)s->N * s->H, 8)), dim3(256), 0, (hipStream_t)stream, *s, *dst, ddst,
                       (const float*)nullptr, out_slope, dsrcs[i], accumulate[i], nob);
  }
  LHN_CHECK_LAUNCH("lhn_ew_bwd");
  return 0;
}
static int bns_of(const lhn_bnsum* in, const lhn_view* v, lhn_bnsum* out, const char* who) {
  memset(out, 0, sizeof(*out));
  if (!in || !in->sums) return 0;
  LHN_CHECK_ARG(in->save && in->C > 0 && in->coff >= 0 && in->coff % 4 == 0 && in->coff + v->C <= in->C && !v->gate && v->table,
                "%s: BatchNorm sums need an ungated input view with a table, inside the producer's %d channels (offset %d, view %d)", who,
                in->C, in->coff, v->C);
  *out = *in;
  return 0;
}
int lhn_ew_bwd2(const lhn_view* src, const lhn_view* dst, const float* ddst, const float* dst_dpool, float out_slope,
                float* dsrc, int accumulate, void* stream) {
  return lhn_ew_bwd3(src, dst, ddst, dst_dpool, out_slope, dsrc, accumulate, nullptr, stream);
}
int lhn_ew_bwd3(const lhn_view* src, const lhn_view* dst, const float* ddst, const float* dst_dpool, float out_slope,
                float* dsrc, int accumulate, const lhn_bnsum* bns, void* stream) {
  LHN_CHECK_ARG(lhn_view_ok(src) && lhn_view_ok(dst) && ddst && dsrc && src->C == dst->C && lhn_no_pend(src) && lhn_no_pend(dst), "lhn_ew_bwd2: bad args");
  LHN_CHECK_ARG(dst->H % src->H == 0 && dst->W % src->W == 0, "lhn_ew_bwd2: non-integer upsample");
  LHN_CHECK_ARG((out_slope != LHN_SLOPE_SILU && out_slope != LHN_SLOPE_RELU_SIGMOID) || (dst->H == src->H && dst->W == src->W), "lhn_ew_bwd2: SiLU / ReLU-sigmoid need a single same-size source");
  LHN_CHECK_ARG(src->C % 4 == 0 && src->C <= 1024, "lhn_ew_bwd2: C=%d", src->C);
  lhn_bnsum bs;
  if (bns_of(bns, src, &bs, "lhn_ew_bwd3")) return 1;
  hipLaunchKernelGGL(k_ew_bwd_src, dim3(grid_cap((int64_t)src->N * src->H, 8)), dim3(256), 0, (hipStream_t)stream, *src, *dst, ddst,
                     dst_dpool, out_slope, dsrc, accumulate, bs);
  LHN_CHECK_LAUNCH("lhn_ew_bwd2");
  return 0;
}

int lhn_ew_bwd_multi(const lhn_view* srcs, int nsrc, const lhn_view* dst, const float* ddst, const float* dst_dpool, float out_slope,
                     float* const* dsrcs, const int* accumulate, const lhn_bnsum* const* bns, void* stream) {
  LHN_CHECK_ARG(srcs && nsrc >= 1 && nsrc <= 3 && lhn_view_ok(dst) && ddst && dsrcs && accumulate && lhn_no_pend(dst), "lhn_ew_bwd_multi: bad args");
  LHN_CHECK_ARG(out_slope != LHN_SLOPE_SILU && out_slope != LHN_SLOPE_RELU_SIGMOID, "lhn_ew_bwd_multi: SiLU / ReLU-sigmoid take lhn_ew_bwd3");
  LHN_CHECK_ARG(dst->C % 4 == 0 && dst->C <= 1024, "lhn_ew_bwd_multi: C=%d", dst->C);
  EwBwdMulti m;
  memset(&m, 0, sizeof(m));
  m.n = nsrc;
  for (int k = 0; k < nsrc; ++k) {
    const lhn_view* v = &srcs[k];
    LHN_CHECK_ARG(lhn_view_ok(v) && lhn_no_pend(v) && dsrcs[k] && v->C == dst->C && v->N == dst->N && v->H == dst->H && v->W == dst->W,
                  "lhn_ew_bwd_multi: source %d must have the destination's geometry", k);
    m.src[k] = *v;
    m.dsrc[k] = dsrcs[k];
    m.acc[k] = accumulate[k];
    if (bns_of(bns ? bns[k] : nullptr, v, &m.bs[k], "lhn_ew_bwd_multi")) return 1;
  }
  hipLaunchKernelGGL(k_ew_bwd_multi, dim3(grid_cap((int64_t)dst->N * dst->H, 8)), dim3(256), 0, (hipStream_t)stream, m, *dst, ddst, dst_dpool, out_slope);
  LHN_CHECK_LAUNCH("lhn_ew_bwd_multi");
  return 0;
}

int lhn_maxpool2_fwd(const lhn_view* x, const lhn_view* y, void* stream) {
  LHN_CHECK_ARG(lhn_view_ok(x) && lhn_view_ok(y) && x->C == y->C, "lhn_maxpool2_fwd: bad views");
  LHN_CHECK_ARG(y->H == (x->H + 1) / 2 && y->W == (x->W + 1) / 2 && y->N == x->N, "lhn_maxpool2_fwd: geometry");
  LHN_CHECK_ARG(y->C % 4 == 0 && y->C <= 1024, "lhn_maxpool2_fwd: C=%d", y->C);
  LHN_CHECK_ARG(lhn_no_pend(x), "lhn_maxpool2_fwd: lhn_view.pend is reserved (NULL)");
  hipLaunchKernelGGL(k_maxpool2_fwd, dim3(grid_cap((int64_t)y->N * y->H, 8)), dim3(256), 0, (hipStream_t)stream, *x, *y);
  LHN_CHECK_LAUNCH("lhn_maxpool2_fwd");
  return 0;
}
int lhn_maxpool2_bwd(const lhn_view* x, const lhn_view* y, const float* dy, float* dx, int dx_accumulate, void* stream) {
  return lhn_maxpool2_bwd2(x, y, dy, dx, dx_accumulate, nullptr, stream);
}
int lhn_maxpool2_bwd2(const lhn_view* x, const lhn_view* y, const float* dy, float* dx, int dx_accumulate, const lhn_bnsum* bns,
                      void* stream) {
  return lhn_maxpool2_bwd3(x, y, dy, dx, dx_accumulate, bns, nullptr, stream);
}
int lhn_maxpool2_bwd3(const lhn_view* x, const lhn_view* y, const float* dy, float* dx, int dx_accumulate, const lhn_bnsum* bns,
                      const lhn_grad_adds* adds, void* stream) {
  LHN_CHECK_ARG(lhn_view_ok(x) && lhn_view_ok(y) && dy && dx && x->C == y->C && lhn_no_pend(x), "lhn_maxpool2_bwd: bad args");
  LHN_CHECK_ARG(y->C % 4 == 0 && y->C <= 1024, "lhn_maxpool2_bwd: C=%d", y->C);
  lhn_bnsum bs;
  if (bns_of(bns, x, &bs, "lhn_maxpool2_bwd2")) return 1;
  lhn_grad_adds ad;
  memset(&ad, 0, sizeof(ad));
  if (adds && (adds->same || adds->pooled)) {
    ad = *adds;
    LHN_CHECK_ARG(x->H % 2 == 0 && x->W % 2 == 0 && y->H == x->H / 2 && y->W == x->W / 2, "lhn_maxpool2_bwd3: gradient addends need even H, W (%dx%d)", x->H, x->W);
    LHN_CHECK_ARG(!ad.same || (ad.same_cstride % 4 == 0 && ad.same_coff % 4 == 0 && ad.same_coff >= 0 && ad.same_coff + x->C <= ad.same_cstride),
                  "lhn_maxpool2_bwd3: same-resolution addend layout");
    LHN_CHECK_ARG(!ad.pooled || (ad.OH > 0 && ad.OW > 0 && ad.OH <= x->H && ad.OW <= x->W && ad.pooled_cstride % 4 == 0 && ad.pooled_coff % 4 == 0 &&
                                 ad.pooled_coff >= 0 && ad.pooled_coff + x->C <= ad.pooled_cstride),
                  "lhn_maxpool2_bwd3: pooled addend layout");
    hipLaunchKernelGGL(k_maxpool2_bwd<true>, dim3(grid_cap((int64_t)y->N * y->H, 8)), dim3(256), 0, (hipStream_t)stream, *x, *y, dy, dx, dx_accumulate, bs, ad);
  } else {
    hipLaunchKernelGGL(k_maxpool2_bwd<false>, dim3(grid_cap((int64_t)y->N * y->H, 8)), dim3(256), 0, (hipStream_t)stream, *x, *y, dy, dx, dx_accumulate, bs, ad);
  }
  LHN_CHECK_LAUNCH("lhn_maxpool2_bwd");
  return 0;
}

int lhn_avgpool_fwd(const lhn_view* x, float* out, int OH, int OW, void* stream) {
  return lhn_avgpool_fwd2(x, out, OH, OW, x ? x->C : 0, 0, stream);
}
int lhn_avgpool_fwd2(const lhn_view* x, float* out, int OH, int OW, int out_cstride, int out_coff, void* stream) {
  LHN_CHECK_ARG(lhn_view_ok(x) && out && OH > 0 && OW > 0 && out_coff >= 0 && out_coff % 4 == 0 && out_cstride % 4 == 0 &&
                    out_coff + x->C <= out_cstride,
                "lhn_avgpool_fwd: bad args");
  LHN_CHECK_ARG(x->C % 4 == 0 && x->C <= 1024, "lhn_avgpool_fwd: C=%d", x->C);
  LHN_CHECK_ARG(lhn_no_pend(x), "lhn_avgpool_fwd: lhn_view.pend is reserved (NULL)");
  const int binmax = ((x->H + OH - 1) / OH + 1) * ((x->W + OW - 1) / OW + 1);
  if (binmax <= 25) {
    const int64_t total = (int64_t)x->N * OH * OW * (x->C / 4);
    hipLaunchKernelGGL(k_avgpool_small, dim3(grid_cap((total + 255) / 256, 16)), dim3(256), 0, (hipStream_t)stream, *x, out, OH, OW, out_cstride, out_coff);
  } else
  {
    BnSlices sl;
    memset(&sl, 0, sizeof(sl));
// ... 207 lines not shown
```

### litehandnet_amd/csrc/lhn_common.h

```cpp
#pragma once
#include <hip/hip_runtime.h>
#include <stdint.h>
#include <stdio.h>
#include <string.h>
#include <mutex>
#include "../../include/lhn.h"

#define LHN_WAVE 64
#define LHN_DEAD (1 << 30)
#define LHN_LANE0(pl, PL) ((pl) < (PL) ? (pl) : LHN_DEAD)

void lhn_set_error(const char* fmt, ...);

#define LHN_CHECK_ARG(cond, ...)                 \
  do {                                           \
    if (!(cond)) {                               \
      lhn_set_error(__VA_ARGS__);                \
      return 1;                                  \
    }                                            \
  } while (0)

#define LHN_CHECK_LAUNCH(name)                                                    \
  do {                                                                            \
    hipError_t e__ = hipGetLastError();                                           \
// ... 446 lines not shown
}

struct TileStat {
  float k, s, q;
  int n;
  __device__ __forceinline__ void reset() { n = 0; k = s = q = 0.f; }
  __device__ __forceinline__ void add(float v) {
    if (n == 0) k = v;
    const float d = v - k;
    s += d;
    q += d * d;
    ++n;
  }
  __device__ __forceinline__ void flush(double& sum, double& sq) const {
    const double K = (double)k, S = (double)s;
    sum += S + (double)n * K;
    sq += (double)q + 2.0 * K * S + (double)n * K * K;
  }
};

__device__ __forceinline__ void lhn_unshift4(double (&sd)[4], double (&qd)[4], f4 s, f4 q, f4 k, int n) {
  const float sv[4] = {s.x, s.y, s.z, s.w}, qv[4] = {q.x, q.y, q.z, q.w}, kv[4] = {k.x, k.y, k.z, k.w};
#pragma unroll
  for (int j = 0; j < 4; ++j) {
    const double K = (double)kv[j], S = (double)sv[j];
    sd[j] += S + (double)n * K;
    qd[j] += (double)qv[j] + 2.0 * K * S + (double)n * K * K;
  }
}

__device__ __forceinline__ void lhn_block_stat_atomics_d(const double (&s)[4], const double (&q)[4], int C4, double* red,
                                                         double* st0, double* st1, int nvalid = 64) {
  double v[8] = {s[0], s[1], s[2], s[3], q[0], q[1], q[2], q[3]};
  for (int o = C4; o < 64; o <<= 1) {
#pragma unroll
    for (int i = 0; i < 8; ++i) v[i] += __shfl_xor(v[i], o, 64);
  }
  const int tid = threadIdx.x, lane = tid & 63, wave = tid >> 6;
  __syncthreads();
  if (lane < C4) {
#pragma unroll
    for (int i = 0; i < 8; ++i) red[(wave * C4 + lane) * 8 + i] = v[i];
  }
  __syncthreads();
  if (tid < 8 * C4) {
    const int kind = tid / (4 * C4), r = tid - kind * 4 * C4, cc = r >> 2, jj = r & 3;
    double t = 0;
#pragma unroll
    for (int wv = 0; wv < 4; ++wv) t += red[(wv * C4 + cc) * 8 + kind * 4 + jj];
    if (cc < nvalid) atomicAdd((kind ? st1 : st0) + 4 * cc + jj, t);
  }
}

__device__ __forceinline__ void lhn_bns_flush(const lhn_bnsum& b, f4 s, f4 q, int C4, f4* red) {
  double* st = b.sums + (size_t)(blockIdx.x % LHN_STAT_REPLICAS) * 2 * b.C + b.coff;
  if (C4 <= 32 && (C4 & (C4 - 1)) == 0) {
    lhn_block_stat_atomics(s, q, C4, red, st, st + b.C);
  } else {
    const int PL = 256 / C4;
    __syncthreads();
    red[threadIdx.x * 2] = s;
    red[threadIdx.x * 2 + 1] = q;
    __syncthreads();
    if ((int)threadIdx.x < C4) {
      double sd[4] = {0, 0, 0, 0}, qd[4] = {0, 0, 0, 0};
      for (int j = 0; j < PL; ++j) {
        const f4 a = red[(j * C4 + threadIdx.x) * 2], c = red[(j * C4 + threadIdx.x) * 2 + 1];
        sd[0] += a.x; sd[1] += a.y; sd[2] += a.z; sd[3] += a.w;
        qd[0] += c.x; qd[1] += c.y; qd[2] += c.z; qd[3] += c.w;
      }
#pragma unroll
      for (int j = 0; j < 4; ++j) {
        atomicAdd(st + 4 * threadIdx.x + j, sd[j]);
        atomicAdd(st + b.C + 4 * threadIdx.x + j, qd[j]);
      }
    }
  }
}
__device__ __forceinline__ f4 lhn_dact_xf(f4 raw, const Xf4& t) {
  const f4 u = raw * t.sc + t.sh;
  return (f4){u.x > 0.f ? 1.f : t.sl.x, u.y > 0.f ? 1.f : t.sl.y, u.z > 0.f ? 1.f : t.sl.z, u.w > 0.f ? 1.f : t.sl.w};
}

__device__ __forceinline__ float lhn_wave_sum(float v) {
#pragma unroll
  for (int o = 32; o > 0; o >>= 1) v += __shfl_xor(v, o, 64);
  return v;
}
__device__ __forceinline__ double lhn_wave_sum_d(double v) {
#pragma unroll
  for (int o = 32; o > 0; o >>= 1) v += __shfl_xor(v, o, 64);
  return v;
}
#endif
```

### litehandnet_amd/csrc/lhn_plan.cpp

```cpp
#include <stdint.h>
#include <stdlib.h>
#include <string.h>
#include <vector>
#include "lhn_common.h"

static lhn_bnsum mkbns(void* ws, int64_t sums_off, int64_t save_off, int C, int coff) {
  lhn_bnsum b;
  memset(&b, 0, sizeof(b));
  if (sums_off >= 0 && save_off >= 0 && C > 0) {
    b.sums = reinterpret_cast<double*>(static_cast<char*>(ws) + sums_off);
    b.save = reinterpret_cast<const float*>(static_cast<char*>(ws) + save_off);
    b.C = C;
    b.coff = coff;
  }
  return b;
}

enum {
  OP_STEM = 1, OP_PW = 2, OP_DW = 3, OP_KXK = 4, OP_FINALIZE = 5, OP_EW = 6, OP_MAXPOOL = 7, OP_AVGPOOL = 8,
  OP_CA_MLP = 9, OP_TABLE_FILL = 10, OP_MEMSET = 11, OP_ATT_MLP = 12, OP_SE_MLP = 13, OP_SHUFFLE = 14,
  OP_PWDW = 15, OP_DWPW = 16, OP_MSRB = 17, OP_CBAM = 18, OP_BNECK = 19,
  OP_STEM_BWD = 101, OP_PW_BWD = 102, OP_DW_BWD = 103, OP_KXK_BWD = 104, OP_BN_BWD = 105, OP_EW_BWD = 106,
  OP_MAXPOOL_BWD = 107, OP_AVGPOOL_BWD = 108, OP_GATE_REDUCE = 109, OP_CA_MLP_BWD = 110, OP_ATT_MLP_BWD = 111, OP_SE_MLP_BWD = 112,
  OP_SHUFFLE_BWD = 113, OP_CBAM_BWD = 114,
};

struct GraphEntry {
  int phase, training, nrep, seen;
  int64_t rstr;
  void *ws, *io0, *io1;
  uint64_t phash, ghash;
  hipGraphExec_t exec;
  uint64_t last_use;
};

struct Plan {
  std::vector<lhn_buf> bufs;
  std::vector<lhn_op> fwd, bwd;
  std::vector<GraphEntry> graphs;
  uint64_t tick = 0;
  int graph_misses = 0;
};

static inline char* at(void* ws, int64_t off) { return off < 0 ? nullptr : static_cast<char*>(ws) + off; }

static lhn_view mkview(const Plan* P, void* ws, int buf, int coff, int C, bool with_gate = true) {
  const lhn_buf& b = P->bufs[buf];
  lhn_view v;
  v.pend = nullptr;
  v.data = reinterpret_cast<float*>(at(ws, b.data_off));
  v.table = reinterpret_cast<const float*>(at(ws, b.table_off));
  v.gate = with_gate ? reinterpret_cast<const float*>(at(ws, b.gate_off)) : nullptr;
  v.N = b.N; v.H = b.H; v.W = b.W;
  v.cstride = b.C; v.coff = coff; v.C = C;
  return v;
}
static lhn_gradview mkgrad(const Plan* P, void* ws, int buf, bool use_coef) {
  const lhn_buf& b = P->bufs[buf];
  lhn_gradview g;
  g.dz = reinterpret_cast<const float*>(at(ws, b.grad_off));
  g.dpool = reinterpret_cast<const float*>(at(ws, b.dpool_off));
  g.coef = use_coef ? reinterpret_cast<const float*>(at(ws, b.coef_off)) : nullptr;
  return g;
}
template <typename T>
static inline T* prm(void* const* arr, int idx) { return idx < 0 ? nullptr : static_cast<T*>(arr[idx]); }
static lhn_bn_slices mkslices(void* ws, const int32_t* pk, const int64_t* sv, const int64_t* sm) {
  lhn_bn_slices s;
  memset(&s, 0, sizeof(s));
  for (int k = 0; k < 2; ++k)
    if (pk[k] > 0 && sv[k] >= 0) {
      const int j = s.n++;
      s.lo[j] = pk[k] >> 16;
      s.C[j] = pk[k] & 0xffff;
      s.save[j] = reinterpret_cast<const float*>(at(ws, sv[k]));
      s.sums[j] = (sm && sm[k] >= 0) ? reinterpret_cast<double*>(at(ws, sm[k])) : nullptr;
    }
  return s;
}

static bool conv_has_bn(const lhn_op& o) { return o.p[2] >= 0 || o.p[3] >= 0 || o.ws[1] >= 0; }
static lhn_bnfin mkfin(const Plan* P, void* ws, const lhn_op& o, void* const* params) {
  const lhn_buf& b = P->bufs[o.out_buf];
  lhn_bnfin f;
  f.counter = reinterpret_cast<uint32_t*>(at(ws, o.ws[2]));
  f.gamma = prm<const float>(params, o.p[2]);
  f.beta = prm<const float>(params, o.p[3]);
  f.running_mean = prm<float>(params, o.p[4]);
  f.running_var = prm<float>(params, o.p[5]);
  f.num_batches_tracked = prm<int64_t>(params, o.p[6]);
  f.table = reinterpret_cast<float*>(at(ws, b.table_off));
  f.save_mean_invstd = reinterpret_cast<float*>(at(ws, o.ws[1]));
  f.count = (double)b.N * b.H * b.W;
  f.cstride = b.C; f.coff = o.out_coff; f.C = o.out_C;
  f.eps = o.f[0]; f.momentum = o.f[1]; f.slope = o.f[2];
  f.conv_bias = prm<const float>(params, o.p[1]);
  return f;
}
static bool fuse_finalize() {
  static int v = -1;
  if (v < 0) {
    const char* e = getenv("LHN_FUSE_FINALIZE");
    v = (e && e[0] == '1') ? 1 : 0;
  }
  return v == 1;
}
static bool bwd_fin_consumer() {
  static int v = -1;
  if (v < 0) {
    const char* e = getenv("LHN_BWD_FIN_CONSUMER");
    v = (e && e[0] == '0') ? 0 : 1;
  }
  return v == 1;
}
bool lhn_head_stream_on();
static bool head_gate_fold_at(const Plan* P, const std::vector<lhn_op>& ops, size_t oi) {
  if (!lhn_head_stream_on() || lhn_deterministic_mode() || oi + 1 >= ops.size()) return false;
  const lhn_op &o = ops[oi], &nx = ops[oi + 1];
  if (o.kind != OP_PW_BWD || !o.i[1] || o.i[0] != 1 || o.i[2] != 1 || o.in_buf[0] < 0) return false;
  if (o.in_C[0] != 128 || o.out_C > 32 || o.i[3] || o.i[4]) return false;
  const lhn_buf& b = P->bufs[o.in_buf[0]];
  return o.in_coff[0] == 0 && o.in_C[0] == b.C && b.gate_off >= 0 && nx.kind == OP_GATE_REDUCE && nx.out_buf == o.in_buf[0] &&
         nx.out_coff == 0 && nx.out_C == b.C && nx.ws[3] >= 0 && nx.ws[4] >= 0;
}

static int sep_finalize(const lhn_bnfin& f, const double* stats, int training, void* stream, int creal = 0, int repeat = 1) {
  int rc = 0;
  for (int r = 0; r < (training ? (repeat < 1 ? 1 : repeat) : 1) && !rc; ++r)
    rc = lhn_bn_finalize2(training ? stats : nullptr, f.gamma, f.beta, f.running_mean, f.running_var,
                          training ? f.num_batches_tracked : nullptr, f.table, f.cstride, f.coff, creal > 0 ? creal : f.C, f.C,
                          training ? f.save_mean_invstd : nullptr, f.count, f.eps, f.momentum, f.slope, training, f.conv_bias, stream);
  return rc;
}

extern "C" {

void* lhn_plan_create(const lhn_buf* bufs, int nbufs, const lhn_op* fwd, int nfwd, const lhn_op* bwd, int nbwd) {
  if (!bufs || nbufs <= 0 || !fwd || nfwd <= 0) {
    lhn_set_error("lhn_plan_create: empty plan");
    return nullptr;
  }
  Plan* p = new Plan();
  p->bufs.assign(bufs, bufs + nbufs);
  p->fwd.assign(fwd, fwd + nfwd);
  if (bwd && nbwd > 0) p->bwd.assign(bwd, bwd + nbwd);
  for (const auto* lst : {&p->fwd, &p->bwd})
    for (const lhn_op& o : *lst) {
      bool ok = o.out_buf < nbufs;
      for (int k = 0; k < 3; ++k) ok = ok && o.in_buf[k] < nbufs;
      if (!ok) {
        lhn_set_error("lhn_plan_create: op kind %d references buffer out of range", o.kind);
        delete p;
        return nullptr;
      }
    }
  return p;
}

int lhn_plan_head_gate_fold(void* plan) {
  const Plan* p = static_cast<const Plan*>(plan);
  if (!p) return -1;
  for (size_t oi = 0; oi + 1 < p->bwd.size(); ++oi)
    if (head_gate_fold_at(p, p->bwd, oi)) return (int)oi + 1;
  return -1;
}

void lhn_plan_destroy(void* plan) {
  Plan* p = static_cast<Plan*>(plan);
  if (!p) return;
  for (GraphEntry& g : p->graphs)
    if (g.exec) (void)hipGraphExecDestroy(g.exec);
  delete p;
}

static int run_ops(const Plan* P, int phase, void* ws, void* const* params, void* const* grads, void* const* io, int mode,
                   int nrep, int64_t rstr, void* stream, size_t sb = 0, size_t se = (size_t)-1, double cscale = 1.0,
                   float pscale = 1.f) {
  const int training = mode & 1;
  const bool skip_tables = (mode & 2) != 0 && !training;
  const std::vector<lhn_op>& ops = phase == 0 ? P->fwd : P->bwd;
  hipStream_t s = static_cast<hipStream_t>(stream);
  int rc = 0;
  const bool whole = (sb == 0 && se >= 2 * ops.size());
  lhn_bnbwdsrc cfin;
  size_t cfin_for = (size_t)-1;
  size_t gfold_at = (size_t)-1;
  for (size_t oi = 0; oi < ops.size() && rc == 0; ++oi) {
    const lhn_op& o = ops[oi];
    const bool deferred = false;
    const bool is_conv = o.kind == OP_STEM || o.kind == OP_PW || o.kind == OP_DW || o.kind == OP_KXK;
    const bool fz = is_conv && training && fuse_finalize() && whole && !(o.kind == OP_PW && o.i[2] > 0) &&
                    !((o.kind == OP_PW || o.kind == OP_DW) && (int)o.f[3] > 1);
    const bool h0 = 2 * oi >= sb && 2 * oi < se, h1 = 2 * oi + 1 >= sb && 2 * oi + 1 < se;
    if (!h0 && !h1) continue;
    const bool two_half = o.kind == OP_STEM || o.kind == OP_PW || o.kind == OP_DW || o.kind == OP_KXK || o.kind == OP_CA_MLP ||
                          o.kind == OP_ATT_MLP || o.kind == OP_BN_BWD || o.kind == OP_CA_MLP_BWD || o.kind == OP_ATT_MLP_BWD;
    if (!two_half && !h0) continue;
    const int stage = (h0 && h1) ? 0 : (h0 ? 1 : 2);
    switch (o.kind) {
      case OP_MEMSET: {
        if (hipMemsetAsync(at(ws, o.ws[0]), 0, (size_t)o.ws[1], s) != hipSuccess) {
          lhn_set_error("lhn_plan_run: memset failed");
          rc = 2;
        }
        break;
      }
      case OP_TABLE_FILL: {
        if (skip_tables) break;
        const lhn_buf& b = P->bufs[o.out_buf];
        if (o.i[0])
          rc = lhn_table_bias(reinterpret_cast<float*>(at(ws, b.table_off)), b.C, o.out_coff, o.out_C, prm<const float>(params, o.p[0]), o.f[2], stream);
        else
          rc = lhn_table_fill(reinterpret_cast<float*>(at(ws, b.table_off)), b.C, o.out_coff, o.out_C, o.f[0], o.f[1], o.f[2], stream);
        break;
      }
      case OP_STEM: {
        lhn_view y = mkview(P, ws, o.out_buf, o.out_coff, o.out_C);
        const bool bn = conv_has_bn(o);
        lhn_bnfin fin;
        if (bn) {
          fin = mkfin(P, ws, o, params);
          fin.count *= cscale;
        }
        if (h0) rc = lhn_conv_stem_fwd(static_cast<const float*>(io[0]), prm<const float>(params, o.p[0]), &y,
                               (training && o.ws[0] >= 0) ? reinterpret_cast<double*>(at(ws, o.ws[0])) : nullptr, o.i[3], o.i[4], o.i[0], o.i[1],
                               o.i[2], (bn && fz) ? &fin : nullptr, stream);
        if (!rc && bn && h1 && !skip_tables && !deferred && !fz) rc = sep_finalize(fin, reinterpret_cast<const double*>(at(ws, o.ws[0])), training, stream);
        break;
      }
      case OP_PW: {
        lhn_view x = mkview(P, ws, o.in_buf[0], o.in_coff[0], o.in_C[0]);
        lhn_view y;
        float* nchw = nullptr;
        if (o.i[1]) {
          y = x;
          y.data = nullptr; y.table = nullptr; y.gate = nullptr; y.pend = nullptr;
          y.cstride = o.out_C; y.coff = 0; y.C = o.out_C;
          nchw = static_cast<float*>(io[1]);
        } else {
          y = mkview(P, ws, o.out_buf, o.out_coff, o.out_C);
        }
        const bool bn = !o.i[1] && conv_has_bn(o);
        lhn_bnfin fin;
        if (bn) {
          fin = mkfin(P, ws, o, params);
          fin.count *= cscale;
        }
        lhn_pw_opts po;
        memset(&po, 0, sizeof(po));
        po.w_rows = o.i[2]; po.w_cols = o.i[3];
        lhn_view extra[2];
        if (o.i[6] > 1) {
          po.n_extra = o.i[6] - 1;
          for (int e = 0; e < po.n_extra; ++e) {
            extra[e] = mkview(P, ws, o.in_buf[e + 1], o.in_coff[e + 1], o.in_C[e + 1]);
          }
          po.extra = extra;
          for (int e = 0; e < 3; ++e) po.coef[e] = o.f[4 + e];
        }
        lhn_view sumv;
        if (o.i[6] > 1 && o.ws[4] >= 0) {
          sumv = x;
          sumv.data = reinterpret_cast<float*>(at(ws, o.ws[4]));
          sumv.table = nullptr; sumv.gate = nullptr; sumv.pend = nullptr;
          sumv.cstride = (int)(o.ws[5] >> 16); sumv.coff = (int)(o.ws[5] & 0xffff);
          po.sum_out = &sumv;
        }
        if (nchw && o.i[5] > 1) {
          const int64_t khw = (int64_t)o.out_C * y.H * y.W;
// ... 152 lines not shown
        break;
      }
      case OP_AVGPOOL: {
        lhn_view x = mkview(P, ws, o.in_buf[0], o.in_coff[0], o.in_C[0], o.i[2] == 0);
        if (o.ws[1] >= 0 || o.in_buf[1] >= 0) {
          const lhn_bn_slices sl = mkslices(ws, &o.i[5], &o.ws[2], nullptr);
          lhn_view src;
          if (o.in_buf[1] >= 0) src = mkview(P, ws, o.in_buf[1], o.in_coff[1], o.in_C[1]);
          rc = lhn_avgpool_fwd4(&x, reinterpret_cast<float*>(at(ws, o.ws[0])), o.i[0], o.i[1],
                                o.ws[1] >= 0 ? reinterpret_cast<float*>(at(ws, o.ws[1])) : nullptr, &sl, o.in_buf[1] >= 0 ? &src : nullptr, stream);
          break;
        }
        rc = lhn_avgpool_fwd2(&x, reinterpret_cast<float*>(at(ws, o.ws[0])), o.i[0], o.i[1], o.i[3] > 0 ? o.i[3] : x.C, o.i[4], stream);
        break;
      }
      case OP_CA_MLP: {
        const lhn_buf& b = P->bufs[o.out_buf];
        if ((!training || o.ws[3] < 0) && !h0) break;
        rc = lhn_ca_mlp_fwd(reinterpret_cast<const float*>(at(ws, o.ws[0])), prm<const float>(params, o.p[0]),
                            prm<const float>(params, o.p[1]), prm<const float>(params, o.p[2]), prm<float>(params, o.p[3]),
                            prm<float>(params, o.p[4]), prm<int64_t>(params, o.p[5]), prm<const float>(params, o.p[6]),
                            prm<const float>(params, o.p[7]), prm<const float>(params, o.p[8]), prm<const float>(params, o.p[9]),
                            (training && o.ws[2] >= 0) ? reinterpret_cast<const float*>(at(ws, o.ws[2])) : nullptr,
                            reinterpret_cast<float*>(at(ws, b.gate_off)), b.C, o.out_coff,
                            reinterpret_cast<float*>(at(ws, o.ws[1])), b.N, o.out_C, o.f[0], o.f[1], training,
                            (training && o.ws[3] >= 0) ? stage : 0, o.ws[3] >= 0 ? reinterpret_cast<double*>(at(ws, o.ws[3])) : nullptr,
                            cscale, stream);
        break;
      }
      case OP_ATT_MLP: {
        const lhn_buf& b = P->bufs[o.out_buf];
        if ((!training || o.ws[3] < 0) && !h0) break;
        rc = lhn_att_mlp_fwd(reinterpret_cast<const float*>(at(ws, o.ws[0])), prm<const float>(params, o.p[0]),
                             prm<const float>(params, o.p[1]), prm<float>(params, o.p[2]), prm<float>(params, o.p[3]),
                             prm<int64_t>(params, o.p[4]), prm<const float>(params, o.p[5]), prm<const float>(params, o.p[6]),
                             prm<const float>(params, o.p[7]), prm<const float>(params, o.p[8]),
                             (training && o.ws[2] >= 0) ? reinterpret_cast<const float*>(at(ws, o.ws[2])) : nullptr,
                             reinterpret_cast<float*>(at(ws, b.gate_off)), b.C, o.out_coff,
                             reinterpret_cast<float*>(at(ws, o.ws[1])), b.N, o.out_C, o.f[0], o.f[1], training,
                             (training && o.ws[3] >= 0) ? stage : 0, o.ws[3] >= 0 ? reinterpret_cast<double*>(at(ws, o.ws[3])) : nullptr,
                             cscale, stream);
        break;
      }
      case OP_SE_MLP: {
        const lhn_buf& b = P->bufs[o.out_buf];
        rc = lhn_se_mlp_fwd2(reinterpret_cast<const float*>(at(ws, o.ws[0])), prm<const float>(params, o.p[0]),
                             prm<const float>(params, o.p[1]), prm<const float>(params, o.p[2]), prm<const float>(params, o.p[3]),
                             reinterpret_cast<float*>(at(ws, b.gate_off)), b.C, o.out_coff, reinterpret_cast<float*>(at(ws, o.ws[1])),
                             b.N, o.out_C, o.i[0], o.i[1], stream);
        break;
      }
      case OP_STEM_BWD: {
        lhn_view y = mkview(P, ws, o.out_buf, o.out_coff, o.out_C);
        lhn_gradview g = mkgrad(P, ws, o.out_buf, o.i[5] != 0);
        rc = lhn_conv_stem_bwd(static_cast<const float*>(io[0]), &y, &g, prm<float>(grads, o.p[1]), o.i[3], o.i[4], o.i[0],
                               o.i[1], o.i[2], nrep, rstr, stream);
        break;
      }
      case OP_PW_BWD: {
        lhn_view x = mkview(P, ws, o.in_buf[0], o.in_coff[0], o.in_C[0]);
        lhn_view y;
        lhn_gradview g;
        const float* nchw = nullptr;
        if (o.i[1]) {
          y = x;
          y.data = nullptr; y.table = nullptr; y.gate = nullptr;
          y.cstride = o.out_C; y.coff = 0; y.C = o.out_C;
          g.dz = nullptr; g.dpool = nullptr; g.coef = nullptr;
          nchw = static_cast<const float*>(io[1]);
        } else {
          y = mkview(P, ws, o.out_buf, o.out_coff, o.out_C);
          g = mkgrad(P, ws, o.out_buf, o.i[5] != 0);
        }
        float* dx = o.i[2] ? reinterpret_cast<float*>(at(ws, P->bufs[o.in_buf[0]].grad_off)) : nullptr;
        lhn_pw_opts po;
        memset(&po, 0, sizeof(po));
        po.w_rows = o.i[3]; po.w_cols = o.i[4];
        if (nchw && o.i[7] > 1) {
          const int64_t khw = (int64_t)o.out_C * y.H * y.W;
          nchw += (int64_t)o.i[6] * khw;
          po.nchw_batch_stride = (int64_t)o.i[7] * khw;
        }
        const lhn_bnsum bs = mkbns(ws, o.ws[0], o.ws[1], (int)o.f[6], (int)o.f[7]);
        lhn_gatesum gsum;
        lhn_bn_slices gsl;
        memset(&gsum, 0, sizeof(gsum));
        if (phase == 1 && whole && head_gate_fold_at(P, ops, oi)) {
          const lhn_op& nx = ops[oi + 1];
          gsl = mkslices(ws, &nx.i[0], &nx.ws[5], nullptr);
          gsum.dgate = reinterpret_cast<float*>(at(ws, nx.ws[3]));
          gsum.slices = &gsl;
          gfold_at = oi + 1;
        }
        rc = lhn_conv_pw_bwd5(&x, prm<const float>(params, o.p[0]), &y, &g, dx, o.i[2] == 2, prm<float>(grads, o.p[1]),
                              prm<float>(grads, o.p[2]), o.i[0], nchw, nrep, rstr, &po, bs.sums ? &bs : nullptr,
                              cfin_for == oi ? &cfin : nullptr, gsum.dgate ? &gsum : nullptr, stream);
        break;
      }
      case OP_DW_BWD: {
        lhn_view x = mkview(P, ws, o.in_buf[0], o.in_coff[0], o.in_C[0]);
        lhn_view y = mkview(P, ws, o.out_buf, o.out_coff, o.out_C);
        lhn_gradview g = mkgrad(P, ws, o.out_buf, o.i[5] != 0);
        float* dx = o.i[4] ? reinterpret_cast<float*>(at(ws, P->bufs[o.in_buf[0]].grad_off)) : nullptr;
        if (cfin_for == oi) {
          const bool adds = o.ws[2] >= 0 || o.ws[3] >= 0;
          const lhn_bnsum bs = mkbns(ws, adds ? -1 : o.ws[4], adds ? -1 : o.ws[5], o.i[6], o.i[7]);
          rc = lhn_conv_dw_bwd4(&x, prm<const float>(params, o.p[0]), &y, &g, dx, o.i[4] == 2, prm<float>(grads, o.p[1]), o.i[0], o.i[1],
                                o.i[2], o.i[3], nrep, rstr, bs.sums ? &bs : nullptr,
                                o.ws[2] >= 0 ? reinterpret_cast<const float*>(at(ws, o.ws[2])) : nullptr,
                                o.ws[3] >= 0 ? reinterpret_cast<const float*>(at(ws, o.ws[3])) : nullptr, &cfin, stream);
          break;
        }
        if (o.ws[2] >= 0 || o.ws[3] >= 0) {
          rc = lhn_conv_dw_bwd3(&x, prm<const float>(params, o.p[0]), &y, &g, dx, o.i[4] == 2, prm<float>(grads, o.p[1]), o.i[0], o.i[1],
                                o.i[2], o.i[3], nrep, rstr, o.ws[2] >= 0 ? reinterpret_cast<const float*>(at(ws, o.ws[2])) : nullptr,
                                o.ws[3] >= 0 ? reinterpret_cast<const float*>(at(ws, o.ws[3])) : nullptr, stream);
          break;
        }
        rc = lhn_conv_dw_bwd2(&x, prm<const float>(params, o.p[0]), &y, &g, dx, o.i[4] == 2, prm<float>(grads, o.p[1]), o.i[0],
                              o.i[1], o.i[2], o.i[3], nrep, rstr, o.ws[4] >= 0 ? reinterpret_cast<double*>(at(ws, o.ws[4])) : nullptr,
                              o.ws[5] >= 0 ? reinterpret_cast<const float*>(at(ws, o.ws[5])) : nullptr, o.i[6], o.i[7], stream);
        break;
      }
      case OP_KXK_BWD: {
        lhn_view x = mkview(P, ws, o.in_buf[0], o.in_coff[0], o.in_C[0]);
        lhn_view y = mkview(P, ws, o.out_buf, o.out_coff, o.out_C);
        lhn_gradview g = mkgrad(P, ws, o.out_buf, o.i[5] != 0);
        float* dx = o.i[2] ? reinterpret_cast<float*>(at(ws, P->bufs[o.in_buf[0]].grad_off)) : nullptr;
        rc = lhn_conv_kxk_bwd(&x, prm<const float>(params, o.p[0]), &y, &g, dx, o.i[2] == 2, prm<float>(grads, o.p[1]), o.i[0],
                              nrep, rstr, o.ws[3] >= 0 ? reinterpret_cast<float*>(at(ws, o.ws[3])) : nullptr, stream);
        break;
      }
      case OP_BN_BWD: {
        const lhn_buf& b = P->bufs[o.out_buf];
        lhn_view y = mkview(P, ws, o.out_buf, o.out_coff, o.out_C);
        lhn_gradview g = mkgrad(P, ws, o.out_buf, false);
        double* sums = reinterpret_cast<double*>(at(ws, o.ws[0]));
        const float* save = reinterpret_cast<const float*>(at(ws, o.ws[1]));
        lhn_bnbwdfin fin;
        fin.counter = reinterpret_cast<uint32_t*>(at(ws, o.ws[2]));
        fin.gamma = prm<const float>(params, o.p[0]);
        fin.coef = reinterpret_cast<float*>(at(ws, b.coef_off));
        fin.dgamma = prm<float>(grads, o.p[1]);
        fin.dbeta = prm<float>(grads, o.p[2]);
        fin.count = (double)b.N * b.H * b.W * cscale;
        fin.cstride = b.C; fin.coff = o.out_coff; fin.C = o.out_C;
        if (fin.counter && fuse_finalize() && whole && !o.i[1]) {
          rc = lhn_bn_bwd_reduce(&y, &g, save, sums, &fin, stream);
        } else {
          if (h0 && !o.i[1]) rc = lhn_bn_bwd_reduce(&y, &g, save, sums, nullptr, stream);
          const lhn_op* nx = oi + 1 < ops.size() ? &ops[oi + 1] : nullptr;
          if (!rc && h1 && whole && bwd_fin_consumer() && !fuse_finalize() && o.i[0] == 0 && nx &&
              (nx->kind == OP_DW_BWD || (nx->kind == OP_PW_BWD && !nx->i[1])) && nx->out_buf == o.out_buf && nx->out_coff == o.out_coff &&
              nx->out_C == o.out_C && nx->i[5] != 0) {
            cfin.sums = sums;
            cfin.save_mean_invstd = save;
            cfin.gamma = fin.gamma;
            cfin.dgamma = fin.dgamma;
            cfin.dbeta = fin.dbeta;
            cfin.count = fin.count;
            cfin.pgrad_scale = pscale;
            cfin.stat_channels = o.out_C;
            cfin_for = oi + 1;
          } else if (!rc && h1)
            rc = lhn_bn_bwd_finalize2(sums, fin.gamma, save, fin.coef, b.C, o.out_coff, o.i[0] > 0 ? o.i[0] : o.out_C, o.out_C, fin.count,
                                      fin.dgamma, fin.dbeta, pscale, stream);
        }
        break;
      }
      case OP_EW_BWD: {
        lhn_view src = mkview(P, ws, o.in_buf[0], o.in_coff[0], o.in_C[0]);
        lhn_view d = mkview(P, ws, o.out_buf, o.out_coff, o.out_C);
        const lhn_buf& db = P->bufs[o.out_buf];
        if (o.i[1] == 1) {
          lhn_view other = mkview(P, ws, o.in_buf[1], o.in_coff[1], o.in_C[1]);
          rc = lhn_ew_mul_bwd(&src, &other, &d, reinterpret_cast<const float*>(at(ws, db.grad_off)),
                              reinterpret_cast<float*>(at(ws, P->bufs[o.in_buf[0]].grad_off)), o.i[0], stream);
        } else if (o.i[1] == 2) {
          rc = lhn_bilinear_bwd(&src, &d, reinterpret_cast<const float*>(at(ws, db.grad_off)),
                                reinterpret_cast<float*>(at(ws, P->bufs[o.in_buf[0]].grad_off)), o.i[0], o.f[0], stream);
        } else if (o.i[1] == 3) {
          lhn_view srcs[3];
          float* dsrcs[3];
          int acc[3] = {o.i[0], o.i[2], o.i[3]};
          lhn_bnsum bsv[3] = {mkbns(ws, o.ws[0], o.ws[1], o.i[4], o.i[5]), mkbns(ws, o.ws[2], o.ws[3], o.i[6], o.i[7]),
                              mkbns(ws, o.ws[4], o.ws[5], (int)o.f[4], (int)o.f[5])};
          const lhn_bnsum* bsp[3];
          int ns = 0;
          for (; ns < 3 && o.in_buf[ns] >= 0; ++ns) {
            srcs[ns] = mkview(P, ws, o.in_buf[ns], o.in_coff[ns], o.in_C[ns]);
            dsrcs[ns] = reinterpret_cast<float*>(at(ws, P->bufs[o.in_buf[ns]].grad_off));
            bsp[ns] = bsv[ns].sums ? &bsv[ns] : nullptr;
          }
          rc = lhn_ew_bwd_multi(srcs, ns, &d, reinterpret_cast<const float*>(at(ws, db.grad_off)),
                                reinterpret_cast<const float*>(at(ws, db.dpool_off)), o.f[0], dsrcs, acc, bsp, stream);
        } else {
          const lhn_bnsum bs = mkbns(ws, o.ws[0], o.ws[1], o.i[4], o.i[5]);
          rc = lhn_ew_bwd3(&src, &d, reinterpret_cast<const float*>(at(ws, db.grad_off)),
                           reinterpret_cast<const float*>(at(ws, db.dpool_off)), o.f[0],
                           reinterpret_cast<float*>(at(ws, P->bufs[o.in_buf[0]].grad_off)), o.i[0], bs.sums ? &bs : nullptr, stream);
        }
        break;
      }
      case OP_MAXPOOL_BWD: {
        lhn_view x = mkview(P, ws, o.in_buf[0], o.in_coff[0], o.in_C[0]);
        lhn_view y = mkview(P, ws, o.out_buf, o.out_coff, o.out_C);
        const lhn_bnsum bs = mkbns(ws, o.ws[0], o.ws[1], o.i[4], o.i[5]);
        lhn_grad_adds ad;
        memset(&ad, 0, sizeof(ad));
        if (o.ws[2] >= 0) {
          ad.same = reinterpret_cast<const float*>(at(ws, o.ws[2]));
          ad.same_cstride = o.i[1]; ad.same_coff = o.i[2];
        }
        if (o.ws[3] >= 0) {
          ad.pooled = reinterpret_cast<const float*>(at(ws, o.ws[3]));
          ad.pooled_cstride = o.i[3]; ad.pooled_coff = o.i[6];
          ad.OH = o.i[7] >> 16; ad.OW = o.i[7] & 0xffff;
        }
        rc = lhn_maxpool2_bwd3(&x, &y, reinterpret_cast<const float*>(at(ws, P->bufs[o.out_buf].grad_off)),
                               reinterpret_cast<float*>(at(ws, P->bufs[o.in_buf[0]].grad_off)), o.i[0], bs.sums ? &bs : nullptr,
                               (ad.same || ad.pooled) ? &ad : nullptr, stream);
        break;
      }
      case OP_AVGPOOL_BWD: {
        lhn_view x = mkview(P, ws, o.in_buf[0], o.in_coff[0], o.in_C[0]);
        const lhn_bnsum bs = mkbns(ws, o.ws[1], o.ws[2], o.i[5], o.i[6]);
        rc = lhn_avgpool_bwd3(&x, reinterpret_cast<const float*>(at(ws, o.ws[0])), o.i[0], o.i[1], o.i[3] > 0 ? o.i[3] : x.C, o.i[4],
                              reinterpret_cast<float*>(at(ws, P->bufs[o.in_buf[0]].grad_off)), o.i[2], bs.sums ? &bs : nullptr, stream);
        break;
      }
      case OP_SHUFFLE_BWD: {
        lhn_view a = mkview(P, ws, o.in_buf[0], o.in_coff[0], o.in_C[0]);
        lhn_view b = mkview(P, ws, o.in_buf[1], o.in_coff[1], o.in_C[1]);
        lhn_view d = mkview(P, ws, o.out_buf, o.out_coff, o.out_C);
        rc = lhn_shuffle2_bwd(&a, &b, &d, reinterpret_cast<const float*>(at(ws, P->bufs[o.out_buf].grad_off)),
                              o.i[0] ? reinterpret_cast<float*>(at(ws, P->bufs[o.in_buf[0]].grad_off)) : nullptr, o.i[0] == 2,
                              o.i[1] ? reinterpret_cast<float*>(at(ws, P->bufs[o.in_buf[1]].grad_off)) : nullptr, o.i[1] == 2, stream);
        break;
      }
      case OP_GATE_REDUCE: {
        if (gfold_at == oi) break;
        lhn_view y = mkview(P, ws, o.out_buf, o.out_coff, o.out_C, false);
        float* dg = reinterpret_cast<float*>(at(ws, o.ws[3]));
        const lhn_bn_slices sl = mkslices(ws, &o.i[0], &o.ws[5], nullptr);
        rc = lhn_gate_bwd_reduce3(&y, reinterpret_cast<const float*>(at(ws, P->bufs[o.out_buf].grad_off)), dg,
                                  o.ws[4] >= 0 ? dg + (size_t)y.N * y.C : nullptr, &sl, 1, stream);
        break;
      }
      case OP_CA_MLP_BWD: {
        const lhn_buf& b = P->bufs[o.out_buf];
        if (o.ws[4] < 0 && !h0) break;
        const lhn_bn_slices sl = mkslices(ws, &o.i[0], &o.ws[6], &o.ws[8]);
        const float* dgp = reinterpret_cast<const float*>(at(ws, o.ws[3]));
        rc = lhn_ca_mlp_bwd2(reinterpret_cast<const float*>(at(ws, o.ws[0])), prm<const float>(params, o.p[0]),
                            prm<const float>(params, o.p[1]), prm<const float>(params, o.p[2]), prm<const float>(params, o.p[3]),
                            o.ws[2] >= 0 ? reinterpret_cast<const float*>(at(ws, o.ws[2])) : nullptr,
                            reinterpret_cast<const float*>(at(ws, o.ws[1])), reinterpret_cast<const float*>(at(ws, o.ws[3])),
                            reinterpret_cast<float*>(at(ws, b.dpool_off)), b.C, o.out_coff, b.H, b.W, prm<float>(grads, o.p[4]),
                            prm<float>(grads, o.p[5]), prm<float>(grads, o.p[6]), prm<float>(grads, o.p[7]),
                            prm<float>(grads, o.p[8]), prm<float>(grads, o.p[9]), prm<float>(grads, o.p[10]), b.N, o.out_C,
                            o.ws[4] >= 0 ? stage : 0, o.ws[4] >= 0 ? reinterpret_cast<double*>(at(ws, o.ws[4])) : nullptr, cscale, pscale,
                            o.ws[5] >= 0 ? dgp + (size_t)b.N * b.C : nullptr, o.ws[5] >= 0 ? reinterpret_cast<const float*>(at(ws, o.ws[5])) : nullptr,
                            &sl, stream);
        break;
      }
      case OP_ATT_MLP_BWD: {
        const lhn_buf& b = P->bufs[o.out_buf];
        if (o.ws[4] < 0 && !h0) break;
        rc = lhn_att_mlp_bwd(reinterpret_cast<const float*>(at(ws, o.ws[0])), prm<const float>(params, o.p[0]),
                             prm<const float>(params, o.p[1]), prm<const float>(params, o.p[2]), prm<const float>(params, o.p[3]),
                             o.ws[2] >= 0 ? reinterpret_cast<const float*>(at(ws, o.ws[2])) : nullptr,
                             reinterpret_cast<float*>(at(ws, o.ws[1])), reinterpret_cast<const float*>(at(ws, o.ws[3])),
                             reinterpret_cast<float*>(at(ws, b.dpool_off)), b.C, o.out_coff, b.H, b.W, prm<float>(grads, o.p[4]),
                             prm<float>(grads, o.p[5]), prm<float>(grads, o.p[6]), prm<float>(grads, o.p[7]),
                             prm<float>(grads, o.p[8]), prm<float>(grads, o.p[9]), b.N, o.out_C,
                             o.ws[4] >= 0 ? stage : 0, o.ws[4] >= 0 ? reinterpret_cast<double*>(at(ws, o.ws[4])) : nullptr, cscale, pscale,
                             stream);
        break;
      }
      case OP_SE_MLP_BWD: {
        const lhn_buf& b = P->bufs[o.out_buf];
        rc = lhn_se_mlp_bwd2(reinterpret_cast<const float*>(at(ws, o.ws[0])), prm<const float>(params, o.p[0]),
                             prm<const float>(params, o.p[1]), reinterpret_cast<const float*>(at(ws, o.ws[1])),
                             reinterpret_cast<const float*>(at(ws, o.ws[3])), reinterpret_cast<float*>(at(ws, b.dpool_off)), b.C,
                             o.out_coff, b.H, b.W, prm<float>(grads, o.p[2]), prm<float>(grads, o.p[3]), prm<float>(grads, o.p[4]),
                             prm<float>(grads, o.p[5]), b.N, o.out_C, o.i[0], o.i[1], stream);
        break;
      }
      case OP_CBAM: {
        lhn_view p = mkview(P, ws, o.in_buf[0], o.in_coff[0], o.in_C[0]), r = mkview(P, ws, o.in_buf[1], o.in_coff[1], o.in_C[1]);
        lhn_view y = mkview(P, ws, o.out_buf, o.out_coff, o.out_C);
        rc = lhn_cbam_fwd(&p, &r, prm<const float>(params, o.p[0]), prm<const float>(params, o.p[1]), prm<const float>(params, o.p[2]),
                          &y, reinterpret_cast<float*>(at(ws, o.ws[0])), stream);
        break;
      }
      case OP_CBAM_BWD: {
        lhn_view p = mkview(P, ws, o.in_buf[0], o.in_coff[0], o.in_C[0]), r = mkview(P, ws, o.in_buf[1], o.in_coff[1], o.in_C[1]);
        lhn_view y = mkview(P, ws, o.out_buf, o.out_coff, o.out_C);
        rc = lhn_cbam_bwd(&p, &r, prm<const float>(params, o.p[0]), prm<const float>(params, o.p[1]), prm<const float>(params, o.p[2]),
                          &y, reinterpret_cast<const float*>(at(ws, P->bufs[o.out_buf].grad_off)),
                          reinterpret_cast<float*>(at(ws, P->bufs[o.in_buf[0]].grad_off)),
                          reinterpret_cast<float*>(at(ws, P->bufs[o.in_buf[1]].grad_off)), prm<float>(grads, o.p[3]),
                          prm<float>(grads, o.p[4]), prm<float>(grads, o.p[5]), reinterpret_cast<const float*>(at(ws, o.ws[0])),
                          reinterpret_cast<float*>(at(ws, o.ws[1])), stream);
        break;
      }
      default:
        lhn_set_error("lhn_plan_run: unknown op kind %d at index %zu", o.kind, oi);
        rc = 1;
    }
  }
  return rc;
}

int lhn_plan_run_range(void* plan, int phase, int64_t step_begin, int64_t step_end, void* ws, void* const* params,
                       void* const* grads, void* const* io, int training, int grad_replicas, int64_t grad_rep_stride,
                       double count_scale, float pgrad_scale, void* stream) {
  LHN_CHECK_ARG(plan && ws && params && io && step_begin >= 0 && step_end >= step_begin && count_scale >= 1, "lhn_plan_run_range: bad argument");
  LHN_CHECK_ARG(phase == 0 || (phase == 1 && grads), "lhn_plan_run_range: phase %d", phase);
  return run_ops(static_cast<const Plan*>(plan), phase, ws, params, grads, io, training, grad_replicas < 1 ? 1 : grad_replicas,
                 grad_rep_stride, stream, (size_t)step_begin, (size_t)step_end, count_scale, pgrad_scale);
}

static bool graphs_enabled() {
// ... 91 lines not shown
```

Measured before the change: 9000 images/s.

## Fold channel-attention gate reductions into the reading pointwise and elementwise backward kernels

Generalizes the head-only gate fold: at plan creation it finds each gate-reduce op whose input buffer is fully covered by 64->64 pointwise-backward or same-size elementwise-backward readers, and has those readers accumulate the dgate and BN-term sums inside their own epilogues via per-sample flushes and atomics. The standalone gate-reduce pass, which re-reads the activation and gradient tensors, is then skipped. In exchange the pointwise kernel uses contiguous tile chunks per block with extra LDS for raw inputs, and partial sums are combined by float atomics, which makes the result order-dependent. It is disabled in deterministic mode or when LHN_GATE_FOLD=0.

After: 9064 images/s, median of 6. Within noise of the previous version (+0.7%).

```diff
diff --git a/include/lhn.h b/include/lhn.h
--- a/include/lhn.h
+++ b/include/lhn.h
@@ -276,6 +276,10 @@
                       const lhn_grad_adds* adds , void* stream);
 int lhn_ew_bwd3(const lhn_view* src, const lhn_view* dst, const float* ddst, const float* dst_dpool, float out_slope, float* dsrc,
                 int accumulate, const lhn_bnsum* bns, void* stream);
+struct lhn_gatesum;
+int lhn_ew_bwd4(const lhn_view* src, const lhn_view* dst, const float* ddst, const float* dst_dpool, float out_slope, float* dsrc,
+                int accumulate, const lhn_bnsum* bns, const struct lhn_gatesum* gs, void* stream);
+int lhn_ew_bwd_gate_folds(int C, int same_res);
 int lhn_ew_bwd_multi(const lhn_view* srcs, int nsrc, const lhn_view* dst, const float* ddst, const float* dst_dpool, float out_slope,
                      float* const* dsrcs, const int* accumulate, const lhn_bnsum* const* bns, void* stream);
 int lhn_avgpool_bwd3(const lhn_view* x, const float* dout, int OH, int OW, int out_cstride, int out_coff, float* dx,
@@ -309,6 +313,7 @@
 int lhn_conv_pw_bwd5(const lhn_view* x, const float* w, const lhn_view* y, const lhn_gradview* gy, float* dx, int dx_accumulate,
                      float* dw, float* dbias, int stride, const float* dy_nchw, int nrep, int64_t rep_stride,
                      const lhn_pw_opts* opts, const lhn_bnsum* bns, const lhn_bnbwdsrc* fin, const lhn_gatesum* gs, void* stream);
+int lhn_pw_bwd_gate_folds(int Cin, int Cout, int HW, int stride, int nchw, int w_rows , int w_cols , int has_bns);
 int lhn_avgpool_fwd3(const lhn_view* x, float* out , int OH, int OW, float* pstat ,
                      const lhn_bn_slices* slices, void* stream);
 int lhn_ca_mlp_bwd2(const float* pooled, const float* w3, const float* gamma, const float* w1, const float* w2,
@@ -353,6 +358,7 @@
 void* lhn_plan_create(const lhn_buf* bufs, int nbufs, const lhn_op* fwd, int nfwd, const lhn_op* bwd, int nbwd);
 void  lhn_plan_destroy(void* plan);
 int   lhn_plan_head_gate_fold(void* plan);
+int   lhn_plan_gate_folds(void* plan, int* idx, int cap);
 #define LHN_RUN_TABLES_CURRENT 2
 #define LHN_RUN_GRAPH 4
 int   lhn_plan_run(void* plan, int phase, void* workspace, void* const* params, void* const* grads,
diff --git a/litehandnet_amd/_lib.py b/litehandnet_amd/_lib.py
--- a/litehandnet_amd/_lib.py
+++ b/litehandnet_amd/_lib.py
@@ -43,7 +43,7 @@
     "lhn_loss_balanced_mse_fwd", "lhn_loss_balanced_mse_bwd", "lhn_affine_warp_normalize", "lhn_affine_warp_normalize2", "lhn_random_flip", "lhn_hsv_jitter", "lhn_simdr_encode", "lhn_simdr_loss_fwd", "lhn_simdr_loss_bwd",
     "lhn_conv_pw_fwd", "lhn_conv_pw_fwd2", "lhn_conv_pw_bwd2", "lhn_conv_dw_fwd", "lhn_conv_dw_fwd2", "lhn_conv_dw_fwd3", "lhn_conv_pw_dw3_fwd", "lhn_conv_dw3_pw_fwd", "lhn_msrb_round_scratch_bytes", "lhn_msrb_round_fwd", "lhn_bottleneck_fwd", "lhn_conv_stem_fwd", "lhn_conv_kxk_fwd",
     "lhn_bn_finalize", "lhn_table_fill", "lhn_table_bias", "lhn_fold_bn", "lhn_ew_fwd", "lhn_ew_fwd2", "lhn_ew_fwd3", "lhn_ew_mul_bwd", "lhn_bilinear_bwd", "lhn_shuffle2_fwd", "lhn_shuffle2_bwd", "lhn_bn_finalize2", "lhn_bn_bwd_finalize2", "lhn_maxpool2_fwd", "lhn_avgpool_fwd", "lhn_avgpool_fwd2", "lhn_avgpool_bwd2", "lhn_se_mlp_fwd2", "lhn_se_mlp_bwd2", "lhn_ca_mlp_fwd", "lhn_att_mlp_fwd", "lhn_att_mlp_bwd", "lhn_se_mlp_fwd", "lhn_se_mlp_bwd",
-    "lhn_bn_bwd_reduce", "lhn_bn_bwd_finalize", "lhn_conv_pw_bwd", "lhn_conv_dw_bwd", "lhn_conv_dw_bwd2", "lhn_conv_dw_bwd3", "lhn_conv_dw_bwd4", "lhn_conv_pw_bwd4", "lhn_conv_pw_bwd5", "lhn_plan_head_gate_fold", "lhn_conv_stem_bwd",
+    "lhn_bn_bwd_reduce", "lhn_bn_bwd_finalize", "lhn_conv_pw_bwd", "lhn_conv_dw_bwd", "lhn_conv_dw_bwd2", "lhn_conv_dw_bwd3", "lhn_conv_dw_bwd4", "lhn_conv_pw_bwd4", "lhn_conv_pw_bwd5", "lhn_plan_head_gate_fold", "lhn_plan_gate_folds", "lhn_pw_bwd_gate_folds", "lhn_ew_bwd4", "lhn_ew_bwd_gate_folds", "lhn_conv_stem_bwd",
     "lhn_conv_kxk_bwd", "lhn_ew_bwd", "lhn_ew_bwd2", "lhn_maxpool2_bwd", "lhn_maxpool2_bwd2", "lhn_maxpool2_bwd3", "lhn_ew_bwd3", "lhn_ew_bwd_multi", "lhn_avgpool_bwd3", "lhn_conv_pw_bwd3", "lhn_avgpool_bwd", "lhn_gate_bwd_reduce", "lhn_gate_bwd_reduce2", "lhn_gate_bwd_reduce3", "lhn_adam_step", "lhn_avgpool_fwd3", "lhn_avgpool_fwd4", "lhn_ca_mlp_bwd2",
     "lhn_ca_mlp_bwd", "lhn_reduce_replicas", "lhn_fold_stat_replicas", "lhn_plan_create", "lhn_plan_destroy", "lhn_plan_run", "lhn_plan_run_range",
     "lhn_cbam_layout", "lhn_cbam_fwd", "lhn_cbam_bwd",
diff --git a/litehandnet_amd/csrc/k_conv_head.hip b/litehandnet_amd/csrc/k_conv_head.hip
--- a/litehandnet_amd/csrc/k_conv_head.hip
+++ b/litehandnet_amd/csrc/k_conv_head.hip
@@ -96,12 +96,7 @@
   return 0;
 }
 
-struct HeadGate {
-  float* dgate;
-  float* tsum;
-  const float* save[2];
-  int lo[2], C[2], n;
-};
+typedef LhnGate HeadGate;
 
 template <bool GS>
 __global__ void __launch_bounds__(256, 2) k_head_bwd(lhn_view x, const float* __restrict__ w, const float* __restrict__ dy,
@@ -298,14 +293,6 @@
   HeadGate hg;
   memset(&hg, 0, sizeof(hg));
   if (!gs) return launch_head_bwd<false>(x, w, dy, dx, dx_acc, dw, dbias, cout, HoWo, bstride, nrep, rep_stride, hg, s);
-  hg.dgate = gs->dgate;
-  hg.tsum = gs->dgate + (size_t)x->N * x->cstride;
-  if (gs->slices)
-    for (int k = 0; k < gs->slices->n; ++k) {
-      hg.save[hg.n] = gs->slices->save[k];
-      hg.lo[hg.n] = gs->slices->lo[k];
-      hg.C[hg.n] = gs->slices->C[k];
-      ++hg.n;
-    }
+  hg = lhn_gate_of(gs, x);
   return launch_head_bwd<true>(x, w, dy, dx, dx_acc, dw, dbias, cout, HoWo, bstride, nrep, rep_stride, hg, s);
 }
diff --git a/litehandnet_amd/csrc/k_conv_pw.hip b/litehandnet_amd/csrc/k_conv_pw.hip
--- a/litehandnet_amd/csrc/k_conv_pw.hip
+++ b/litehandnet_amd/csrc/k_conv_pw.hip
@@ -933,10 +933,11 @@
   return launch_pw_bwd_t<CIN, NTO, false>(x, w, y, gy, dx, dx_acc, dw, dbias, stride, dy_nchw, cout, nrep, rep_stride, geo, s, bs);
 }
 
-template <int CIN, int COUT, int PX, int PF, bool DYST, bool BNS, int OCC>
+template <int CIN, int COUT, int PX, int PF, bool DYST, bool BNS, int OCC, bool GS = false>
 __global__ void __launch_bounds__(256, OCC) k_pw_bwd_wr(lhn_view x, const float* __restrict__ w, lhn_view y, lhn_gradview gy,
                                                         float* __restrict__ dx, int dx_acc, float* __restrict__ dw, float* __restrict__ dbias,
-                                                        int M, int ntiles, int nrep, int64_t rep_stride, lhn_bnsum bs, lhn_bnbwdsrc fs) {
+                                                        int M, int ntiles, int nrep, int64_t rep_stride, lhn_bnsum bs, lhn_bnbwdsrc fs,
+                                                        LhnGate hg, int chunk) {
   constexpr int NTI = CIN / 32, NTO = COUT / 32, LDY = COUT + 4, LDX = CIN + 4;
   constexpr bool ONE = NTI == 1;
   constexpr int NDW = ONE ? 1 : NTO * NTI / 4;
@@ -946,6 +947,8 @@
   static_assert(ONE ? (NTO == 1 && PX == 128) : ((NTI == 2 || NTI == 4) && (NTO == 2 || NTO == 4) && (PX == 64 || (PX == 32 && NTI == 4))),
                 "32 -> 32 at 128 pixels; 64 / 128 channels on either side at 64 (or 32) pixels");
   static_assert(!BNS || NDX == 1, "reader-side sums: one dX sub-tile per wave");
+  constexpr int LDR = GS ? CIN + 8 : CIN;
+  static_assert(!GS || (NDX == 1 && !BNS), "gate sums: one dX sub-tile per wave, and not next to the BatchNorm sums (those views are ungated)");
   extern __shared__ __attribute__((aligned(16))) float smem[];
   float* dYs = smem;
   float* Xs = dYs + PX * LDY;
@@ -953,6 +956,7 @@
   float* yt = xt + 3 * CIN;
   float* cf = yt + 3 * COUT;
   float* Xr = cf + 3 * COUT;
+  float* gred = Xr + PX * (CIN + 8);
   const int tid = threadIdx.x, lane = tid & 63, wave = __builtin_amdgcn_readfirstlane(tid >> 6), l31 = lane & 31, lh = lane >> 5;
   const int HoWo = y.H * y.W;
   float* dzw = const_cast<float*>(gy.dz);
@@ -992,7 +996,7 @@
         if (!BNS && x.gate) v *= *reinterpret_cast<const f4*>(x.gate + (int64_t)(m / HoWo) * x.cstride + xabs);
       }
       *reinterpret_cast<f4*>(Xs + row * LDX + 4 * xc4) = v;
-      if (BNS) *reinterpret_cast<f4*>(Xr + row * CIN + 4 * xc4) = m < M ? xraw[p] : (f4){0.f, 0.f, 0.f, 0.f};
+      if (BNS || GS) *reinterpret_cast<f4*>(Xr + row * LDR + 4 * xc4) = m < M ? xraw[p] : (f4){0.f, 0.f, 0.f, 0.f};
     }
     Xf4 yxf;
     Gr4 ygr;
@@ -1031,8 +1035,9 @@
     }
   };
 
-  int tile = blockIdx.x;
-  if (tile < ntiles) issue(tile);
+  const int tstep = GS ? 1 : (int)gridDim.x, tend = GS ? min(ntiles, ((int)blockIdx.x + 1) * chunk) : ntiles;
+  int tile = GS ? blockIdx.x * chunk : blockIdx.x;
+  if (tile < tend) issue(tile);
   static_assert(PX * LDY * sizeof(float) >= 2 * LHN_FIN_THREADS * sizeof(double), "dYs holds the replica fold's partials");
   LhnBwdPre fpre;
   if (fs.sums) {
@@ -1076,6 +1081,38 @@
   }
   double* const bst = BNS ? bs.sums + (size_t)(blockIdx.x % LHN_STAT_REPLICAS) * 2 * bs.C + bs.coff + (tid & (CIN - 1)) : nullptr;
   const int bsC = BNS ? bs.C : 0;
+  const int cg = x.coff + 32 * jt + l31;
+  float g_sc = 1.f, g_sh = 0.f, g_sl = 1.f, g_mean = 0.f, g_inv = 1.f, g_d = 0.f, g_0 = 0.f, g_1 = 0.f;
+  int n_cur = -1;
+  if (GS) {
+    if (x.table) {
+      g_sc = x.table[cg];
+      g_sh = x.table[x.cstride + cg];
+      g_sl = x.table[2 * x.cstride + cg];
+    }
+    lhn_gate_mi(hg, cg, g_mean, g_inv);
+  }
+  auto gflush = [&]() __attribute__((always_inline)) {
+    const float sd = g_d + __shfl_xor(g_d, 32, 64), s0 = g_0 + __shfl_xor(g_0, 32, 64), s1 = g_1 + __shfl_xor(g_1, 32, 64);
+    if (lh == 0) {
+      gred[(wave * 3 + 0) * 32 + l31] = sd;
+      gred[(wave * 3 + 1) * 32 + l31] = s0;
+      gred[(wave * 3 + 2) * 32 + l31] = s1;
+    }
+    __syncthreads();
+    if (tid < CIN && n_cur >= 0) {
+      const int w0 = (tid >> 5) * NWC, c = tid & 31;
+      float v[3] = {0.f, 0.f, 0.f};
+#pragma unroll
+      for (int q = 0; q < NWC; ++q)
+#pragma unroll
+        for (int k = 0; k < 3; ++k) v[k] += gred[((w0 + q) * 3 + k) * 32 + c];
+      atomicAdd(hg.dgate + (int64_t)n_cur * x.cstride + x.coff + tid, v[0]);
+      atomicAdd(hg.tsum + ((int64_t)n_cur * 2 + 0) * x.cstride + x.coff + tid, v[1]);
+      atomicAdd(hg.tsum + ((int64_t)n_cur * 2 + 1) * x.cstride + x.coff + tid, v[2]);
+    }
+    g_d = g_0 = g_1 = 0.f;
+  };
   if (fs.sums) {
     __syncthreads();
     if (tid < COUT)
@@ -1085,10 +1122,10 @@
   }
   __syncthreads();
 
-  for (; tile < ntiles; tile += gridDim.x) {
+  for (; tile < tend; tile += tstep) {
     commit(tile);
     __syncthreads();
-    if (tile + (int)gridDim.x < ntiles) issue(tile + gridDim.x);
+    if (tile + tstep < tend) issue(tile + tstep);
     {
       const float* ap = dYs + ((ONE ? 32 * wave : 0) + lh) * LDY + l31 + (ONE ? 0 : 32 * (wave / NTI));
       const float* bp = Xs + ((ONE ? 32 * wave : 0) + lh) * LDX + l31 + (ONE ? 0 : 32 * (wave % NTI));
@@ -1103,6 +1140,13 @@
       }
     }
     if (dx) {
+      if (GS) {
+        const int n = (tile * PX) / HoWo;
+        if (n != n_cur) {
+          gflush();
+          n_cur = n;
+        }
+      }
       f16v accx[NDX];
 #pragma unroll
       for (int hh = 0; hh < NDX; ++hh)
@@ -1135,6 +1179,22 @@
             b_q += du * ((raw - b_mean) * b_inv);
           }
         }
+        if (GS) {
+          const float* xr = Xr + ((mt0 + hh) * 32 + 4 * lh) * LDR + 32 * jt + l31;
+          float t_d = 0.f, t_0 = 0.f, t_1 = 0.f;
+#pragma unroll
+          for (int r = 0; r < 16; ++r) {
+            const float raw = xr[((r & 3) + 8 * (r >> 2)) * LDR];
+            const float u = raw * g_sc + g_sh;
+            const float da = accx[hh][r] * (u > 0.f ? 1.f : g_sl);
+            t_d += accx[hh][r] * lhn_lrelu(u, g_sl);
+            t_0 += da;
+            t_1 += da * ((raw - g_mean) * g_inv);
+          }
+          g_d += t_d;
+          g_0 += t_0;
+          g_1 += t_1;
+        }
         if (tile * PX + PX <= M) {
           if (dx_acc) {
 #pragma unroll
@@ -1161,6 +1221,7 @@
     }
     __syncthreads();
   }
+  if (GS) gflush();
 
   if (BNS) {
     float* bred = Xs;
@@ -1222,23 +1283,28 @@
   }
 }
 
-template <int CIN, int COUT, int PX, int PF, bool DYST = true, bool BNS = false, int OCC = 2>
+template <int CIN, int COUT, int PX, int PF, bool DYST = true, bool BNS = false, int OCC = 2, bool GS = false>
 static int launch_pw_bwd_wr(const lhn_view* x, const float* w, const lhn_view* y, const lhn_gradview* gy, float* dx, int dx_acc, float* dw,
-                            float* dbias, int nrep, int64_t rep_stride, hipStream_t s, const lhn_bnsum& bs, const lhn_bnbwdsrc* fsp = nullptr) {
+                            float* dbias, int nrep, int64_t rep_stride, hipStream_t s, const lhn_bnsum& bs, const lhn_bnbwdsrc* fsp = nullptr,
+                            const lhn_gatesum* gs = nullptr) {
   const int M = y->N * y->H * y->W, ntiles = (M + PX - 1) / PX;
   lhn_bnbwdsrc fs;
   if (fsp) fs = *fsp; else memset(&fs, 0, sizeof(fs));
-  const size_t lds = (size_t)(PX * (COUT + 4) + PX * (CIN + 4) + 3 * CIN + 6 * COUT + (BNS ? PX * CIN : 0)) * sizeof(float);
+  const size_t lds = (size_t)(PX * (COUT + 4) + PX * (CIN + 4) + 3 * CIN + 6 * COUT + (BNS ? PX * CIN : GS ? PX * (CIN + 8) + 4 * 3 * 32 : 0)) * sizeof(float);
   static LhnKernelCfg cfg;
   int per_cu = 1;
-  if (!lhn_kernel_cfg(cfg, &k_pw_bwd_wr<CIN, COUT, PX, PF, DYST, BNS, OCC>, lds, OCC, &per_cu)) {
+  if (!lhn_kernel_cfg(cfg, &k_pw_bwd_wr<CIN, COUT, PX, PF, DYST, BNS, OCC, GS>, lds, OCC, &per_cu)) {
     lhn_set_error("lhn_conv_pw_bwd: cannot reserve %zu B of LDS", lds);
     return 2;
   }
-  int grid = lhn_num_cus() * per_cu;
+  int grid = lhn_num_cus() * per_cu, chunk = 1;
   if (grid > ntiles) grid = ntiles;
-  hipLaunchKernelGGL((k_pw_bwd_wr<CIN, COUT, PX, PF, DYST, BNS, OCC>), dim3(grid), dim3(256), lds, s, *x, w, *y, *gy, dx, dx_acc, dw, dbias,
-                     M, ntiles, nrep, rep_stride, bs, fs);
+  if (GS) {
+    chunk = (ntiles + grid - 1) / grid;
+    grid = (ntiles + chunk - 1) / chunk;
+  }
+  hipLaunchKernelGGL((k_pw_bwd_wr<CIN, COUT, PX, PF, DYST, BNS, OCC, GS>), dim3(grid), dim3(256), lds, s, *x, w, *y, *gy, dx, dx_acc, dw, dbias,
+                     M, ntiles, nrep, rep_stride, bs, fs, lhn_gate_of(GS ? gs : nullptr, x), chunk);
   return 0;
 }
 
@@ -1281,6 +1347,10 @@
 static int pw_bwd_run(const lhn_view* x, const float* w, const lhn_view* y, const lhn_gradview* gy, float* dx, int dx_accumulate, float* dw,
                       float* dbias, int stride, const float* dy_nchw, int nrep, int64_t rep_stride, const lhn_pw_opts* opts,
                       const lhn_bnsum* bns, const lhn_bnbwdsrc* fin, const lhn_gatesum* gs, bool* gs_done, void* stream);
+extern "C" int lhn_pw_bwd_gate_folds(int Cin, int Cout, int HW, int stride, int nchw, int w_rows, int w_cols, int has_bns) {
+  return Cin == 64 && Cout == 64 && HW > 0 && HW % 64 == 0 && stride == 1 && !nchw && (w_rows <= 0 || w_rows == Cout) &&
+         (w_cols <= 0 || w_cols == Cin) && !has_bns && !pw_bwd_narrow_off() && !pw_wr_off() && !lhn_deterministic_mode();
+}
 extern "C" int lhn_conv_pw_bwd5(const lhn_view* x, const float* w, const lhn_view* y, const lhn_gradview* gy, float* dx,
                                 int dx_accumulate, float* dw, float* dbias, int stride, const float* dy_nchw, int nrep,
                                 int64_t rep_stride, const lhn_pw_opts* opts, const lhn_bnsum* bns, const lhn_bnbwdsrc* fin,
@@ -1288,6 +1358,10 @@
   if (gs && !gs->dgate) gs = nullptr;
   if (gs) LHN_CHECK_ARG(lhn_view_ok(x) && dx && !dx_accumulate && stride == 1 && (!gs->slices || (gs->slices->n >= 0 && gs->slices->n <= 2)),
                         "lhn_conv_pw_bwd5: gate sums need a stored dx (no accumulate), stride 1 and 0..2 BatchNorm slices");
+  if (gs && (x->coff != 0 || x->C != x->cstride))
+    LHN_CHECK_ARG(y && lhn_pw_bwd_gate_folds(x->C, y->C, x->H * x->W, stride, dy_nchw != nullptr, opts ? opts->w_rows : 0, opts ? opts->w_cols : 0,
+                                             bns && bns->sums),
+                  "lhn_conv_pw_bwd5: gate sums of a channel slice ride in the 64 -> 64 register-W kernel only (see lhn_pw_bwd_gate_folds)");
   bool gs_done = false;
   const int rc = pw_bwd_run(x, w, y, gy, dx, dx_accumulate, dw, dbias, stride, dy_nchw, nrep, rep_stride, opts, bns, fin, gs, &gs_done, stream);
   if (rc || !gs || gs_done) return rc;
@@ -1354,7 +1428,10 @@
   }
   if (wr_narrow) {
     int rc;
-    if (Cin == 64) rc = bs.sums ? launch_pw_bwd_wr<64, 64, 64, 2, false, true>(x, w, y, gy, dx, dx_accumulate, dw, dbias, nrep, rep_stride, s, bs, fin)
+    if (Cin == 64 && gs && lhn_pw_bwd_gate_folds(Cin, Cout, HoWo, stride, 0, wrows, wcols, bs.sums != nullptr)) {
+      rc = launch_pw_bwd_wr<64, 64, 64, 2, false, false, 2, true>(x, w, y, gy, dx, dx_accumulate, dw, dbias, nrep, rep_stride, s, bs, fin, gs);
+      *gs_done = rc == 0;
+    } else if (Cin == 64) rc = bs.sums ? launch_pw_bwd_wr<64, 64, 64, 2, false, true>(x, w, y, gy, dx, dx_accumulate, dw, dbias, nrep, rep_stride, s, bs, fin)
                                 : launch_pw_bwd_wr<64, 64, 64, 2, false, false>(x, w, y, gy, dx, dx_accumulate, dw, dbias, nrep, rep_stride, s, bs, fin);
     else rc = bs.sums ? launch_pw_bwd_wr<32, 32, 128, 2, false, true>(x, w, y, gy, dx, dx_accumulate, dw, dbias, nrep, rep_stride, s, bs, fin)
                       : launch_pw_bwd_wr<32, 32, 128, 2, false, false, 3>(x, w, y, gy, dx, dx_accumulate, dw, dbias, nrep, rep_stride, s, bs, fin);
diff --git a/litehandnet_amd/csrc/k_misc.hip b/litehandnet_amd/csrc/k_misc.hip
--- a/litehandnet_amd/csrc/k_misc.hip
+++ b/litehandnet_amd/csrc/k_misc.hip
@@ -222,14 +222,15 @@
   }
 }
 
+template <bool GS>
 __global__ void __launch_bounds__(256) k_ew_bwd_src(lhn_view src, lhn_view dst, const float* __restrict__ ddst,
                                                     const float* __restrict__ dst_dpool, float out_slope,
-                                                    float* __restrict__ dsrc, int accumulate, lhn_bnsum bs) {
-  __shared__ f4 bred[512];
+                                                    float* __restrict__ dsrc, int accumulate, lhn_bnsum bs, LhnGate hg, int chunk) {
+  __shared__ f4 bred[GS ? 768 : 512];
   const int C4 = src.C >> 2, c4 = threadIdx.x % C4, pl = threadIdx.x / C4, PL = 256 / C4;
   f4 bsum = (f4){0.f, 0.f, 0.f, 0.f}, bsq = bsum, bmean = bsum, binv = bsum;
   Xf4 bxf;
-  if (bs.sums) {
+  if (!GS && bs.sums) {
     bxf = lhn_load_xf(src, src.coff + 4 * c4);
     bmean = *reinterpret_cast<const f4*>(bs.save + bs.coff + 4 * c4);
     binv = *reinterpret_cast<const f4*>(bs.save + bs.C + bs.coff + 4 * c4);
@@ -237,8 +238,44 @@
   const int fh = dst.H / src.H, fw = dst.W / src.W;
   const int cd = dst.coff + 4 * c4;
   const int rows = src.N * src.H;
-  for (int row = blockIdx.x; row < rows; row += gridDim.x) {
+  if (GS) {
+    bxf = lhn_load_xf(src, src.coff + 4 * c4);
+    float m4[4], i4[4];
+#pragma unroll
+    for (int j = 0; j < 4; ++j) lhn_gate_mi(hg, src.coff + 4 * c4 + j, m4[j], i4[j]);
+    bmean = (f4){m4[0], m4[1], m4[2], m4[3]};
+    binv = (f4){i4[0], i4[1], i4[2], i4[3]};
+  }
+  f4 gd = (f4){0.f, 0.f, 0.f, 0.f}, g0 = gd, g1 = gd;
+  int n_cur = -1;
+  auto gflush = [&]() __attribute__((always_inline)) {
+    bred[threadIdx.x] = gd;
+    bred[256 + threadIdx.x] = g0;
+    bred[512 + threadIdx.x] = g1;
+    __syncthreads();
+    if ((int)threadIdx.x < src.C) {
+      const float* rf = reinterpret_cast<const float*>(bred);
+      float t = 0.f, u0 = 0.f, u1 = 0.f;
+      for (int j = 0; j < PL; ++j) {
+        t += rf[j * src.C + threadIdx.x];
+        u0 += rf[1024 + j * src.C + threadIdx.x];
+        u1 += rf[2048 + j * src.C + threadIdx.x];
+      }
+      const int ca = src.coff + threadIdx.x;
+      atomicAdd(hg.dgate + (size_t)n_cur * src.cstride + ca, t);
+      atomicAdd(hg.tsum + ((size_t)n_cur * 2 + 0) * src.cstride + ca, u0);
+      atomicAdd(hg.tsum + ((size_t)n_cur * 2 + 1) * src.cstride + ca, u1);
+    }
+    __syncthreads();
+    gd = g0 = g1 = (f4){0.f, 0.f, 0.f, 0.f};
+  };
+  const int rstep = GS ? 1 : (int)gridDim.x, rend = GS ? min(rows, ((int)blockIdx.x + 1) * chunk) : rows;
+  for (int row = GS ? blockIdx.x * chunk : blockIdx.x; row < rend; row += rstep) {
     const int n = row / src.H, h = row - n * src.H;
+    if (GS && n != n_cur) {
+      if (n_cur >= 0) gflush();
+      n_cur = n;
+    }
     const f4 gate = dst.gate ? *reinterpret_cast<const f4*>(dst.gate + (size_t)n * dst.cstride + cd) : (f4){1.f, 1.f, 1.f, 1.f};
     for (int w = LHN_LANE0(pl, PL); w < src.W; w += PL) {
       f4 g = (f4){0.f, 0.f, 0.f, 0.f};
@@ -275,17 +312,25 @@
           g += e;
         }
       float* o = dsrc + ((size_t)row * src.W + w) * src.cstride + src.coff + 4 * c4;
-      if (bs.sums) {
+      if (!GS && bs.sums) {
         const f4 raw = *reinterpret_cast<const f4*>(src.data + ((size_t)row * src.W + w) * src.cstride + src.coff + 4 * c4);
         const f4 du = g * lhn_dact_xf(raw, bxf);
         bsum += du;
         bsq += du * ((raw - bmean) * binv);
       }
+      if (GS) {
+        const f4 raw = *reinterpret_cast<const f4*>(src.data + ((size_t)row * src.W + w) * src.cstride + src.coff + 4 * c4);
+        const f4 da = g * lhn_dact_xf(raw, bxf);
+        gd += g * lhn_apply_xf(raw, bxf);
+        g0 += da;
+        g1 += da * ((raw - bmean) * binv);
+      }
       if (accumulate) g += *reinterpret_cast<const f4*>(o);
       *reinterpret_cast<f4*>(o) = g;
     }
   }
-  if (bs.sums) lhn_bns_flush(bs, bsum, bsq, C4, bred);
+  if (GS && n_cur >= 0) gflush();
+  if (!GS && bs.sums) lhn_bns_flush(bs, bsum, bsq, C4, bred);
 }
 
 struct EwBwdMulti {
@@ -1179,8 +1224,8 @@
     const lhn_view* s = &srcs[i];
     lhn_bnsum nob;
     memset(&nob, 0, sizeof(nob));
-    hipLaunchKernelGGL(k_ew_bwd_src, dim3(grid_cap((int64_t)s->N * s->H, 8)), dim3(256), 0, (hipStream_t)stream, *s, *dst, ddst,
-                       (const float*)nullptr, out_slope, dsrcs[i], accumulate[i], nob);
+    hipLaunchKernelGGL(k_ew_bwd_src<false>, dim3(grid_cap((int64_t)s->N * s->H, 8)), dim3(256), 0, (hipStream_t)stream, *s, *dst, ddst,
+                       (const float*)nullptr, out_slope, dsrcs[i], accumulate[i], nob, lhn_gate_of(nullptr, s), 0);
   }
   LHN_CHECK_LAUNCH("lhn_ew_bwd");
   return 0;
@@ -1200,14 +1245,32 @@
 }
 int lhn_ew_bwd3(const lhn_view* src, const lhn_view* dst, const float* ddst, const float* dst_dpool, float out_slope,
                 float* dsrc, int accumulate, const lhn_bnsum* bns, void* stream) {
+  return lhn_ew_bwd4(src, dst, ddst, dst_dpool, out_slope, dsrc, accumulate, bns, nullptr, stream);
+}
+int lhn_ew_bwd_gate_folds(int C, int same_res) { return same_res && C > 0 && C % 4 == 0 && C <= 256 && !lhn_deterministic_mode(); }
+int lhn_ew_bwd4(const lhn_view* src, const lhn_view* dst, const float* ddst, const float* dst_dpool, float out_slope,
+                float* dsrc, int accumulate, const lhn_bnsum* bns, const lhn_gatesum* gs, void* stream) {
   LHN_CHECK_ARG(lhn_view_ok(src) && lhn_view_ok(dst) && ddst && dsrc && src->C == dst->C && lhn_no_pend(src) && lhn_no_pend(dst), "lhn_ew_bwd2: bad args");
   LHN_CHECK_ARG(dst->H % src->H == 0 && dst->W % src->W == 0, "lhn_ew_bwd2: non-integer upsample");
   LHN_CHECK_ARG((out_slope != LHN_SLOPE_SILU && out_slope != LHN_SLOPE_RELU_SIGMOID) || (dst->H == src->H && dst->W == src->W), "lhn_ew_bwd2: SiLU / ReLU-sigmoid need a single same-size source");
   LHN_CHECK_ARG(src->C % 4 == 0 && src->C <= 1024, "lhn_ew_bwd2: C=%d", src->C);
   lhn_bnsum bs;
   if (bns_of(bns, src, &bs, "lhn_ew_bwd3")) return 1;
-  hipLaunchKernelGGL(k_ew_bwd_src, dim3(grid_cap((int64_t)src->N * src->H, 8)), dim3(256), 0, (hipStream_t)stream, *src, *dst, ddst,
-                     dst_dpool, out_slope, dsrc, accumulate, bs);
+  if (gs && gs->dgate) {
+    LHN_CHECK_ARG(!accumulate && !bs.sums && lhn_ew_bwd_gate_folds(src->C, dst->H == src->H && dst->W == src->W) &&
+                      (!gs->slices || (gs->slices->n >= 0 && gs->slices->n <= 2)),
+                  "lhn_ew_bwd4: gate sums need a stored dsrc (no accumulate), no bns, a same-size source of <= 256 channels and 0..2 BatchNorm slices");
+    const int rows = src->N * src->H;
+    int grid = grid_cap(rows, 8);
+    const int chunk = (rows + grid - 1) / grid;
+    grid = (rows + chunk - 1) / chunk;
+    hipLaunchKernelGGL(k_ew_bwd_src<true>, dim3(grid), dim3(256), 0, (hipStream_t)stream, *src, *dst, ddst,
+                       dst_dpool, out_slope, dsrc, accumulate, bs, lhn_gate_of(gs, src), chunk);
+    LHN_CHECK_LAUNCH("lhn_ew_bwd4");
+    return 0;
+  }
+  hipLaunchKernelGGL(k_ew_bwd_src<false>, dim3(grid_cap((int64_t)src->N * src->H, 8)), dim3(256), 0, (hipStream_t)stream, *src, *dst, ddst,
+                     dst_dpool, out_slope, dsrc, accumulate, bs, lhn_gate_of(nullptr, src), 0);
   LHN_CHECK_LAUNCH("lhn_ew_bwd2");
   return 0;
 }
diff --git a/litehandnet_amd/csrc/lhn_common.h b/litehandnet_amd/csrc/lhn_common.h
--- a/litehandnet_amd/csrc/lhn_common.h
+++ b/litehandnet_amd/csrc/lhn_common.h
@@ -552,6 +552,38 @@
   return (f4){u.x > 0.f ? 1.f : t.sl.x, u.y > 0.f ? 1.f : t.sl.y, u.z > 0.f ? 1.f : t.sl.z, u.w > 0.f ? 1.f : t.sl.w};
 }
 
+struct LhnGate {
+  float* dgate;
+  float* tsum;
+  const float* save[2];
+  int lo[2], C[2], n;
+};
+static inline LhnGate lhn_gate_of(const lhn_gatesum* gs, const lhn_view* x) {
+  LhnGate g;
+  memset(&g, 0, sizeof(g));
+  if (!gs || !gs->dgate) return g;
+  g.dgate = gs->dgate;
+  g.tsum = gs->dgate + (size_t)x->N * x->cstride;
+  if (gs->slices)
+    for (int k = 0; k < gs->slices->n && k < 2; ++k) {
+      g.save[g.n] = gs->slices->save[k];
+      g.lo[g.n] = gs->slices->lo[k];
+      g.C[g.n] = gs->slices->C[k];
+      ++g.n;
+    }
+  return g;
+}
+__device__ __forceinline__ void lhn_gate_mi(const LhnGate& g, int c, float& mean, float& inv) {
+  mean = 0.f;
+  inv = 1.f;
+#pragma unroll
+  for (int k = 0; k < 2; ++k)
+    if (k < g.n && c >= g.lo[k] && c < g.lo[k] + g.C[k]) {
+      mean = g.save[k][c - g.lo[k]];
+      inv = g.save[k][g.C[k] + c - g.lo[k]];
+    }
+}
+
 __device__ __forceinline__ float lhn_wave_sum(float v) {
 #pragma unroll
   for (int o = 32; o > 0; o >>= 1) v += __shfl_xor(v, o, 64);
diff --git a/litehandnet_amd/csrc/lhn_plan.cpp b/litehandnet_amd/csrc/lhn_plan.cpp
--- a/litehandnet_amd/csrc/lhn_plan.cpp
+++ b/litehandnet_amd/csrc/lhn_plan.cpp
@@ -40,6 +40,8 @@
   std::vector<GraphEntry> graphs;
   uint64_t tick = 0;
   int graph_misses = 0;
+  std::vector<int32_t> gfold_src;
+  std::vector<char> gfold_skip;
 };
 
 static inline char* at(void* ws, int64_t off) { return off < 0 ? nullptr : static_cast<char*>(ws) + off; }
@@ -124,6 +126,63 @@
          nx.out_coff == 0 && nx.out_C == b.C && nx.ws[3] >= 0 && nx.ws[4] >= 0;
 }
 
+static bool gate_fold_on() {
+  static int v = -1;
+  if (v < 0) {
+    const char* e = getenv("LHN_GATE_FOLD");
+    v = (e && e[0] == '0') ? 0 : 1;
+  }
+  return v == 1;
+}
+static void build_gate_folds(Plan* P) {
+  const std::vector<lhn_op>& ops = P->bwd;
+  P->gfold_src.assign(ops.size(), -1);
+  P->gfold_skip.assign(ops.size(), 0);
+  for (size_t oi = 0; oi + 1 < ops.size(); ++oi)
+    if (head_gate_fold_at(P, ops, oi)) {
+      P->gfold_src[oi] = (int32_t)oi + 1;
+      P->gfold_skip[oi + 1] = 1;
+    }
+  if (!gate_fold_on() || lhn_deterministic_mode()) return;
+  for (size_t gi = 0; gi < ops.size(); ++gi) {
+    const lhn_op& g = ops[gi];
+    if (g.kind != OP_GATE_REDUCE || P->gfold_skip[gi] || g.ws[3] < 0 || g.ws[4] < 0 || g.out_buf < 0) continue;
+    const lhn_buf& b = P->bufs[g.out_buf];
+    if (b.gate_off < 0 || g.out_coff != 0 || g.out_C != b.C) continue;
+    std::vector<size_t> readers;
+    std::vector<char> covered(b.C, 0);
+    bool ok = true;
+    for (size_t k = gi; k-- > 0 && ok;) {
+      const lhn_op& o = ops[k];
+      if (o.kind == OP_BN_BWD) continue;
+      if (o.in_buf[0] != g.out_buf || P->gfold_src[k] >= 0) break;
+      bool adds = false;
+      if (o.kind == OP_PW_BWD)
+        adds = !o.i[1] && o.i[0] == 1 && o.i[2] == 1 &&
+               lhn_pw_bwd_gate_folds(o.in_C[0], o.out_C, b.H * b.W, o.i[0], o.i[1], o.i[3], o.i[4], o.ws[0] >= 0 && o.ws[1] >= 0);
+      else if (o.kind == OP_EW_BWD)
+        adds = o.i[1] == 0 && o.i[0] == 0 && o.out_buf >= 0 && P->bufs[o.out_buf].H == b.H && P->bufs[o.out_buf].W == b.W &&
+               !(o.ws[0] >= 0 && o.ws[1] >= 0 && o.i[4] > 0) &&
+               lhn_ew_bwd_gate_folds(o.in_C[0], 1);
+      else
+        break;
+      if (!adds || o.in_coff[0] < 0 || o.in_coff[0] + o.in_C[0] > b.C) {
+        ok = false;
+        break;
+      }
+      for (int c = o.in_coff[0]; c < o.in_coff[0] + o.in_C[0]; ++c) {
+        if (covered[c]) ok = false;
+        covered[c] = 1;
+      }
+      readers.push_back(k);
+    }
+    for (int c = 0; c < b.C && ok; ++c) ok = covered[c] != 0;
+    if (!ok || readers.empty()) continue;
+    for (size_t k : readers) P->gfold_src[k] = (int32_t)gi;
+    P->gfold_skip[gi] = 1;
+  }
+}
+
 static int sep_finalize(const lhn_bnfin& f, const double* stats, int training, void* stream, int creal = 0, int repeat = 1) {
   int rc = 0;
   for (int r = 0; r < (training ? (repeat < 1 ? 1 : repeat) : 1) && !rc; ++r)
@@ -154,7 +213,20 @@
         return nullptr;
       }
     }
+  build_gate_folds(p);
   return p;
+}
+
+int lhn_plan_gate_folds(void* plan, int* idx, int cap) {
+  const Plan* p = static_cast<const Plan*>(plan);
+  if (!p) return -1;
+  int n = 0;
+  for (size_t oi = 0; oi < p->gfold_skip.size(); ++oi)
+    if (p->gfold_skip[oi]) {
+      if (idx && n < cap) idx[n] = (int)oi;
+      ++n;
+    }
+  return n;
 }
 
 int lhn_plan_head_gate_fold(void* plan) {
@@ -184,7 +256,16 @@
   const bool whole = (sb == 0 && se >= 2 * ops.size());
   lhn_bnbwdsrc cfin;
   size_t cfin_for = (size_t)-1;
-  size_t gfold_at = (size_t)-1;
+  lhn_gatesum gsum;
+  lhn_bn_slices gsl;
+  auto gate_sums_of = [&](size_t oi) -> const lhn_gatesum* {
+    if (phase != 1 || !whole || P->gfold_src[oi] < 0) return nullptr;
+    const lhn_op& gr = ops[P->gfold_src[oi]];
+    gsl = mkslices(ws, &gr.i[0], &gr.ws[5], nullptr);
+    gsum.dgate = reinterpret_cast<float*>(at(ws, gr.ws[3]));
+    gsum.slices = &gsl;
+    return &gsum;
+  };
   for (size_t oi = 0; oi < ops.size() && rc == 0; ++oi) {
     const lhn_op& o = ops[oi];
     const bool deferred = false;
@@ -503,19 +584,9 @@
           po.nchw_batch_stride = (int64_t)o.i[7] * khw;
         }
         const lhn_bnsum bs = mkbns(ws, o.ws[0], o.ws[1], (int)o.f[6], (int)o.f[7]);
-        lhn_gatesum gsum;
-        lhn_bn_slices gsl;
-        memset(&gsum, 0, sizeof(gsum));
-        if (phase == 1 && whole && head_gate_fold_at(P, ops, oi)) {
-          const lhn_op& nx = ops[oi + 1];
-          gsl = mkslices(ws, &nx.i[0], &nx.ws[5], nullptr);
-          gsum.dgate = reinterpret_cast<float*>(at(ws, nx.ws[3]));
-          gsum.slices = &gsl;
-          gfold_at = oi + 1;
-        }
         rc = lhn_conv_pw_bwd5(&x, prm<const float>(params, o.p[0]), &y, &g, dx, o.i[2] == 2, prm<float>(grads, o.p[1]),
                               prm<float>(grads, o.p[2]), o.i[0], nchw, nrep, rstr, &po, bs.sums ? &bs : nullptr,
-                              cfin_for == oi ? &cfin : nullptr, gsum.dgate ? &gsum : nullptr, stream);
+                              cfin_for == oi ? &cfin : nullptr, gate_sums_of(oi), stream);
         break;
       }
       case OP_DW_BWD: {
@@ -617,9 +688,10 @@
                                 reinterpret_cast<const float*>(at(ws, db.dpool_off)), o.f[0], dsrcs, acc, bsp, stream);
         } else {
           const lhn_bnsum bs = mkbns(ws, o.ws[0], o.ws[1], o.i[4], o.i[5]);
-          rc = lhn_ew_bwd3(&src, &d, reinterpret_cast<const float*>(at(ws, db.grad_off)),
+          rc = lhn_ew_bwd4(&src, &d, reinterpret_cast<const float*>(at(ws, db.grad_off)),
                            reinterpret_cast<const float*>(at(ws, db.dpool_off)), o.f[0],
-                           reinterpret_cast<float*>(at(ws, P->bufs[o.in_buf[0]].grad_off)), o.i[0], bs.sums ? &bs : nullptr, stream);
+                           reinterpret_cast<float*>(at(ws, P->bufs[o.in_buf[0]].grad_off)), o.i[0], bs.sums ? &bs : nullptr,
+                           gate_sums_of(oi), stream);
         }
         break;
       }
@@ -660,7 +732,7 @@
         break;
       }
       case OP_GATE_REDUCE: {
-        if (gfold_at == oi) break;
+        if (phase == 1 && whole && P->gfold_skip[oi]) break;
         lhn_view y = mkview(P, ws, o.out_buf, o.out_coff, o.out_C, false);
         float* dg = reinterpret_cast<float*>(at(ws, o.ws[3]));
         const lhn_bn_slices sl = mkslices(ws, &o.i[0], &o.ws[5], nullptr);
```
